# eddyxzc/lpopc

Measured on AMD Instinct MI355X. Metric: eval_g+eval_jac_g calls/sec, 4-phase 4096-LGR-pt problem, higher is better.
Workload: dtype f64

## Files before the change

lpopc_amd/csrc/rpm_abi.cpp:

```cpp
#include <cmath>
#include <cstdio>
#include <cstring>
#include <vector>
#include <new>
#include <string>

#include "rpm_engine.hpp"
#include "rpm_pin.h"

static thread_local std::string g_create_error;

using rpm::Engine;

#define RPM_GUARD_BEGIN try {
#define RPM_GUARD_END(eng)                                   \
  }                                                          \
  catch (const std::exception& ex) {                         \
    (eng).err = std::string("internal error: ") + ex.what(); \
    return RPM_E_INVALID;                                    \
  }                                                          \
  catch (...) {                                              \
    (eng).err = "internal error";                            \
    return RPM_E_INVALID;                                    \
  }

static int fail(Engine& e, int code, const char* msg) {
  e.err = msg;
  return code;
}

extern "C" {

int rpm_create(const rpm_problem_desc* desc, rpm_engine** out) {
  if (!out) {
    g_create_error = "rpm_create: out is NULL";
    return RPM_E_INVALID;
  }
  *out = nullptr;
  rpm_engine* h = new (std::nothrow) rpm_engine();
  if (!h) {
    g_create_error = "out of memory";
    return RPM_E_INVALID;
  }
  int rc;
  try {
    rc = rpm::setup_engine(h->e, desc);
  } catch (const std::exception& ex) {
    h->e.err = std::string("internal error: ") + ex.what();
    rc = RPM_E_INVALID;
  }
  if (rc != RPM_OK) {
    g_create_error = h->e.err;
    delete h;
    return rc;
  }
  *out = h;
  return RPM_OK;
}

void rpm_destroy(rpm_engine* h) {
  if (!h) return;
  rpm::device_destroy(h->e);
  delete h;
}

const char* rpm_last_error(const rpm_engine* h) {
  if (!h) return g_create_error.c_str();
  if (h->e.pin_note.empty()) return h->e.err.c_str();
  rpm_engine* w = const_cast<rpm_engine*>(h);
  w->e.err_report = h->e.err + (h->e.err.empty() ? "" : "; ") + "page-lock registry: " + h->e.pin_note;
  return w->e.err_report.c_str();
}

int rpm_device_init(rpm_engine* h, int device_id) {
  if (!h) return RPM_E_INVALID;
  RPM_GUARD_BEGIN
  return rpm::device_init(h->e, device_id);
  RPM_GUARD_END(h->e)
}

int rpm_get_nlp_info(rpm_engine* h, int* n, int* m, int* nnz_jac_g, int* nnz_h_lag, int* index_style) {
  if (!h) return RPM_E_INVALID;
  Engine& e = h->e;
  RPM_GUARD_BEGIN
  if (e.hessian_mode == RPM_HESSIAN_EXACT && nnz_h_lag) {
    int rc = rpm::ensure_hessian(e);
    if (rc) return rc;
  }
  if (n) *n = e.n;
  if (m) *m = e.m;
  if (nnz_jac_g) *nnz_jac_g = e.nnz_jac;
  if (nnz_h_lag) *nnz_h_lag = e.nnz_h;
  if (index_style) *index_style = 0;
  return RPM_OK;
  RPM_GUARD_END(e)
}

int rpm_get_bounds_info(rpm_engine* h, int n, double* x_l, double* x_u, int m, double* g_l, double* g_u) {
  if (!h) return RPM_E_INVALID;
  Engine& e = h->e;
  if (n != e.n || m != e.m || !x_l || !x_u || !g_l || !g_u) return fail(e, RPM_E_INVALID, "get_bounds_info: size mismatch");
  std::memcpy(x_l, e.xl.data(), sizeof(double) * e.n);
  std::memcpy(x_u, e.xu.data(), sizeof(double) * e.n);
  std::memcpy(g_l, e.gl.data(), sizeof(double) * e.m);
  std::memcpy(g_u, e.gu.data(), sizeof(double) * e.m);
  return RPM_OK;
}

int rpm_get_starting_point(rpm_engine* h, int n, int init_x, double* x, int init_z, double* z_L, double* z_U,
                           int m, int init_lambda, double* lambda) {
  (void)z_L; (void)z_U; (void)lambda;
  if (!h) return RPM_E_INVALID;
  Engine& e = h->e;
  if (!init_x || init_z || init_lambda) return fail(e, RPM_E_INVALID, "get_starting_point: only init_x is supported");
  if (n != e.n || m != e.m || !x) return fail(e, RPM_E_INVALID, "get_starting_point: size mismatch");
  std::memcpy(x, e.guess.data(), sizeof(double) * e.n);
  return RPM_OK;
}

static int stage_x(Engine& e, int n, const double* x) {
  if (n != e.n || !x) return fail(e, RPM_E_INVALID, "x size mismatch");
  if (!e.dev) {
    int rc = rpm::device_init(e, 0);
    if (rc) return rc;
  }
  return rpm::dev_upload_x(e, x);
}

int rpm_eval_f(rpm_engine* h, int n, const double* x, int new_x, double* obj_value) {
  if (!h) return RPM_E_INVALID;
  Engine& e = h->e;
  RPM_GUARD_BEGIN
  if (!obj_value) return fail(e, RPM_E_INVALID, "eval_f: obj_value is NULL");
  if (n != e.n || !x) return fail(e, RPM_E_INVALID, "x size mismatch");
  return rpm::host_eval_f(e, x, new_x, obj_value);
  RPM_GUARD_END(e)
}

int rpm_eval_grad_f(rpm_engine* h, int n, const double* x, int new_x, double* grad_f) {
  if (!h) return RPM_E_INVALID;
  Engine& e = h->e;
  RPM_GUARD_BEGIN
  if (!grad_f) return fail(e, RPM_E_INVALID, "eval_grad_f: grad_f is NULL");
  if (n != e.n || !x) return fail(e, RPM_E_INVALID, "x size mismatch");
  return rpm::host_eval_grad_f(e, x, new_x, grad_f);
  RPM_GUARD_END(e)
}

int rpm_eval_g(rpm_engine* h, int n, const double* x, int new_x, int m, double* g) {
  if (!h) return RPM_E_INVALID;
  Engine& e = h->e;
  RPM_GUARD_BEGIN
  if (n != e.n || !x) return fail(e, RPM_E_INVALID, "x size mismatch");
  if (m != e.m || !g) return fail(e, RPM_E_INVALID, "eval_g: size mismatch");
  return rpm::host_eval_g(e, x, new_x, g);
  RPM_GUARD_END(e)
}

int rpm_eval_jac_g(rpm_engine* h, int n, const double* x, int new_x, int m, int nele_jac, int* iRow, int* jCol,
                   double* values) {
  if (!h) return RPM_E_INVALID;
  Engine& e = h->e;
  RPM_GUARD_BEGIN
  if (n != e.n || m != e.m || nele_jac != e.nnz_jac) return fail(e, RPM_E_INVALID, "eval_jac_g: size mismatch");
  if (!values) {
    if (!iRow || !jCol) return fail(e, RPM_E_INVALID, "eval_jac_g: iRow/jCol are NULL in the structure pass");
    std::memcpy(iRow, e.jac_i.data(), sizeof(int) * e.nnz_jac);
    std::memcpy(jCol, e.jac_j.data(), sizeof(int) * e.nnz_jac);
    return RPM_OK;
  }
  if (!x) return fail(e, RPM_E_INVALID, "eval_jac_g: x is NULL");
  return rpm::host_eval_jac_values(e, x, new_x, values);
  RPM_GUARD_END(e)
}

int rpm_eval_pair(rpm_engine* h, int n, const double* x, int m, double* g, int nele_jac, double* values) {
  if (!h) return RPM_E_INVALID;
  Engine& e = h->e;
  RPM_GUARD_BEGIN
  if (n != e.n || m != e.m || nele_jac != e.nnz_jac || !x || !g || !values) return fail(e, RPM_E_INVALID, "eval_pair: size mismatch or NULL pointer");
  return rpm::host_eval_pair(e, x, g, values);
  RPM_GUARD_END(e)
}

int rpm_eval_h(rpm_engine* h, int n, const double* x, int new_x, double obj_factor, int m, const double* lambda,
               int new_lambda, int nele_hess, int* iRow, int* jCol, double* values) {
  (void)new_lambda;
  if (!h) return RPM_E_INVALID;
  Engine& e = h->e;
  RPM_GUARD_BEGIN
  if (e.hessian_mode != RPM_HESSIAN_EXACT) return fail(e, RPM_E_UNSUPPORTED, "eval_h: the engine was created with hessian-approximation=limited-memory");
  int rc = rpm::ensure_hessian(e);
  if (rc) return rc;
  if (n != e.n || m != e.m || nele_hess != e.nnz_h) return fail(e, RPM_E_INVALID, "eval_h: size mismatch");
  if (!values) {
    if (!iRow || !jCol) return fail(e, RPM_E_INVALID, "eval_h: iRow/jCol are NULL in the structure pass");
    std::memcpy(iRow, e.hes_i.data(), sizeof(int) * e.nnz_h);
    std::memcpy(jCol, e.hes_j.data(), sizeof(int) * e.nnz_h);
    return RPM_OK;
  }
  if (!x || !lambda) return fail(e, RPM_E_INVALID, "eval_h: x or lambda is NULL");
  if (new_x) rpm::host_new_x(e);
  rc = stage_x(e, n, x);
  if (rc) return rc;
  rc = rpm::dev_upload(e, rpm::dev_buf(e, 5), lambda, size_t(e.n_instances) * e.m, rpm::STAGE_LAMBDA);
  if (rc) return rc;
  rc = rpm::dev_eval_h(e, rpm::dev_buf(e, 0), obj_factor, rpm::dev_buf(e, 5), rpm::dev_buf(e, 6), rpm::dev_stream(e));
  if (rc) return rc;
  rc = rpm::dev_download(e, values, rpm::dev_buf(e, 6), size_t(e.n_instances) * e.nnz_h, rpm::STAGE_HESS);
  if (rc) return rc;
  if (e.opt_check_finite && rpm::dev_nonfinite(e, rpm::dev_buf(e, 6), size_t(e.n_instances) * e.nnz_h) != 0) return fail(e, RPM_E_NONFINITE, "eval_h: non-finite Hessian value");
  return RPM_OK;
  RPM_GUARD_END(e)
}

int rpm_finalize_solution(rpm_engine* h, int status, int n, const double* x, const double* z_L, const double* z_U,
                          int m, const double* g, const double* lambda, double obj_value) {
  (void)status; (void)z_L; (void)z_U; (void)g;
  if (!h) return RPM_E_INVALID;
  Engine& e = h->e;
  if (n != e.n || m != e.m || !x || !lambda) return fail(e, RPM_E_INVALID, "finalize_solution: size mismatch");
  e.sol_x.assign(x, x + n);
  e.sol_lambda.assign(lambda, lambda + m);
  e.sol_obj = obj_value;
  e.has_solution = true;
  return RPM_OK;
}

int rpm_get_solution(rpm_engine* h, int n, double* x, int m, double* lambda, double* obj_value) {
  if (!h) return RPM_E_INVALID;
  Engine& e = h->e;
  if (!e.has_solution) return fail(e, RPM_E_INVALID, "no solution stored");
  if (n != e.n || m != e.m) return fail(e, RPM_E_INVALID, "get_solution: size mismatch");
  if (x) std::memcpy(x, e.sol_x.data(), sizeof(double) * n);
  if (lambda) std::memcpy(lambda, e.sol_lambda.data(), sizeof(double) * m);
  if (obj_value) *obj_value = e.sol_obj;
  return RPM_OK;
}

int rpm_nlp2op_control(rpm_engine* h, int phase, const double* x, const double* lambda, double* time, double* state,
                       double* control, double* costate, double* pathmult, double* hamiltonian, double* mayer_cost,
                       double* lagrange_cost) {
  if (!h) return RPM_E_INVALID;
  Engine& e = h->e;
  RPM_GUARD_BEGIN
  if (phase < 0 || phase >= e.P) return fail(e, RPM_E_INVALID, "The phase index is out of rang");
  if (e.n_instances != 1) return fail(e, RPM_E_UNSUPPORTED, "nlp2op_control: one instance per engine");
  if (!x || !lambda) {
    if (!e.has_solution) return fail(e, RPM_E_INVALID, "nlp2op_control: no x/lambda given and no solution stored");
    x = e.sol_x.data();
    lambda = e.sol_lambda.data();
  }
  return rpm::dev_nlp2op(e, phase, x, lambda, time, state, control, costate, pathmult, hamiltonian, mayer_cost, lagrange_cost);
  RPM_GUARD_END(e)
}

int rpm_solution_error(rpm_engine* h, int phase, const double* x, double* rel_err, int* rows) {
  if (!h) return RPM_E_INVALID;
  Engine& e = h->e;
  RPM_GUARD_BEGIN
  if (phase < 0 || phase >= e.P) return fail(e, RPM_E_INVALID, "The phase index is out of rang");
  if (e.n_instances != 1) return fail(e, RPM_E_UNSUPPORTED, "solution_error: one instance per engine");
  if (!x) {
    if (!e.has_solution) return fail(e, RPM_E_INVALID, "solution_error: no x given and no solution stored");
    x = e.sol_x.data();
  }
  if (rows) *rows = e.ph[phase].N + e.ph[phase].K + 1;
  if (!rel_err) return RPM_OK;
  return rpm::dev_solution_error(e, phase, x, rel_err);
  RPM_GUARD_END(e)
}

static int refine_from(Engine& e, int phase, const double* rel, double tol, int nmin, int nmax, int capacity,
                       double* new_mesh_points, int* new_nodes_per_interval, int* new_n_intervals, double* interval_error,
                       int* no_more_refine) {
  std::vector<double> mesh, emax;
  std::vector<int> nodes;
  const bool done = rpm::ph_refine(e.ph[phase], rel, tol, nmin, nmax, mesh, nodes, emax);
  if (new_n_intervals) *new_n_intervals = int(nodes.size());
  if (no_more_refine) *no_more_refine = done ? 1 : 0;
  if (interval_error) std::memcpy(interval_error, emax.data(), sizeof(double) * emax.size());
  if (new_mesh_points || new_nodes_per_interval) {
    if (capacity < int(nodes.size())) return fail(e, RPM_E_INVALID, "ph_refine_mesh: capacity is smaller than the new interval count");
    if (new_mesh_points) std::memcpy(new_mesh_points, mesh.data(), sizeof(double) * mesh.size());
    if (new_nodes_per_interval) std::memcpy(new_nodes_per_interval, nodes.data(), sizeof(int) * nodes.size());
  }
  return RPM_OK;
}

int rpm_ph_refine_from_error(rpm_engine* h, int phase, const double* rel_err, double tol, int nmin, int nmax, int capacity,
                             double* new_mesh_points, int* new_nodes_per_interval, int* new_n_intervals,
                             double* interval_error, int* no_more_refine) {
  if (!h) return RPM_E_INVALID;
  Engine& e = h->e;
  RPM_GUARD_BEGIN
  if (phase < 0 || phase >= e.P) return fail(e, RPM_E_INVALID, "The phase index is out of rang");
  if (!rel_err) return fail(e, RPM_E_INVALID, "ph_refine_from_error: rel_err is NULL");
  if (!(tol > 0) || nmin < 2 || nmax < nmin) return fail(e, RPM_E_INVALID, "ph_refine_mesh: need tol > 0 and 2 <= Nmin <= Nmax");
  return refine_from(e, phase, rel_err, tol, nmin, nmax, capacity, new_mesh_points, new_nodes_per_interval, new_n_intervals,
                     interval_error, no_more_refine);
  RPM_GUARD_END(e)
}

int rpm_ph_refine_mesh(rpm_engine* h, int phase, const double* x, double tol, int nmin, int nmax, int capacity,
                       double* new_mesh_points, int* new_nodes_per_interval, int* new_n_intervals,
                       double* interval_error, int* no_more_refine) {
  if (!h) return RPM_E_INVALID;
  Engine& e = h->e;
  RPM_GUARD_BEGIN
  if (phase < 0 || phase >= e.P) return fail(e, RPM_E_INVALID, "The phase index is out of rang");
  if (e.n_instances != 1) return fail(e, RPM_E_UNSUPPORTED, "ph_refine_mesh: one instance per engine");
  if (!(tol > 0) || nmin < 2 || nmax < nmin) return fail(e, RPM_E_INVALID, "ph_refine_mesh: need tol > 0 and 2 <= Nmin <= Nmax");
  if (!x) {
    if (!e.has_solution) return fail(e, RPM_E_INVALID, "ph_refine_mesh: no x given and no solution stored");
    x = e.sol_x.data();
  }
  const rpm::PhaseHost& p = e.ph[phase];
  std::vector<double> rel(size_t(p.N + p.K + 1) * p.nx);
  int rc = rpm::dev_solution_error(e, phase, x, rel.data());
  if (rc) return rc;
  return refine_from(e, phase, rel.data(), tol, nmin, nmax, capacity, new_mesh_points, new_nodes_per_interval,
                     new_n_intervals, interval_error, no_more_refine);
  RPM_GUARD_END(e)
}

int rpm_solution_error_batch_sizes(rpm_engine* h, int* n_intervals_total, long long* rel_doubles_total) {
  if (!h) return RPM_E_INVALID;
  rpm::solution_error_batch_sizes(h->e, n_intervals_total, rel_doubles_total);
  return RPM_OK;
}

int rpm_solution_error_batch_dev(rpm_engine* h, const double* d_x, const int* d_instance_mask, double* d_interval_error,
                                 double* d_rel_err_max, double* d_rel_err, int* d_nonfinite, void* stream) {
  if (!h) return RPM_E_INVALID;
  Engine& e = h->e;
  RPM_GUARD_BEGIN
  if (!d_x) return fail(e, RPM_E_INVALID, "solution_error_batch_dev: d_x is NULL");
  if (e.shard_mode == RPM_SHARD_INTERVALS && e.shard_world > 1) return fail(e, RPM_E_UNSUPPORTED, "solution_error_batch: not with interval sharding");
  return rpm::dev_solution_error_batch(e, d_x, d_instance_mask, d_interval_error, d_rel_err_max, d_rel_err, d_nonfinite, stream);
  RPM_GUARD_END(e)
}

int rpm_solution_error_batch(rpm_engine* h, const double* x, const int* instance_mask, double* interval_error,
                             double* rel_err_max, double* rel_err, int* nonfinite) {
  if (!h) return RPM_E_INVALID;
  Engine& e = h->e;
  RPM_GUARD_BEGIN
  if (!x) return fail(e, RPM_E_INVALID, "solution_error_batch: x is NULL");
  if (e.shard_mode == RPM_SHARD_INTERVALS && e.shard_world > 1) return fail(e, RPM_E_UNSUPPORTED, "solution_error_batch: not with interval sharding");
  if (instance_mask && rel_err_max) {
    bool any = false;
    for (int b = 0; b < e.n_instances; ++b) any = any || instance_mask[b] != 0;
    if (!any) return fail(e, RPM_E_INVALID, "solution_error_batch: rel_err_max asked for, but instance_mask excludes every instance");
  }
  return rpm::host_solution_error_batch(e, x, instance_mask, interval_error, rel_err_max, rel_err, nonfinite);
  RPM_GUARD_END(e)
}

struct rpm_hpliu {
  rpm::HpLiu h;
  int n_phases = 0;
  std::string err;
};

int rpm_hpliu_create(int n_phases, double tol, int nmax, double ratio_r, rpm_hpliu** out) {
  if (!out || n_phases < 1 || !(tol > 0) || nmax < 2 || !(ratio_r > 0)) return RPM_E_INVALID;
  rpm_hpliu* p = new (std::nothrow) rpm_hpliu();
  if (!p) return RPM_E_INVALID;
  p->n_phases = n_phases;
  p->h.tol = tol;
  p->h.Nmax = nmax;
  p->h.R = ratio_r;
  *out = p;
  return RPM_OK;
}

void rpm_hpliu_destroy(rpm_hpliu* p) { delete p; }

const char* rpm_hpliu_last_error(const rpm_hpliu* p) { return p ? p->err.c_str() : "null hp-Liu object"; }

int rpm_hpliu_refine(rpm_hpliu* p, rpm_engine* h, const double* x, const double* rel_err, int capacity,
                     double* new_mesh_points, int* new_nodes_per_interval, int* mesh_off, int* nodes_off,
                     int* new_n_intervals, int* no_more_refine) {
  if (!p || !h) return RPM_E_INVALID;
  Engine& e = h->e;
  RPM_GUARD_BEGIN
  if (e.P != p->n_phases) return fail(e, RPM_E_INVALID, "hpliu_refine: phase count differs from rpm_hpliu_create");
  if (e.n_instances != 1) return fail(e, RPM_E_UNSUPPORTED, "hpliu_refine: one instance per engine");
  if (!x) {
    if (!e.has_solution) return fail(e, RPM_E_INVALID, "hpliu_refine: no x given and no solution stored");
    x = e.sol_x.data();
  }
  std::vector<std::vector<double>> rel(e.P);
  const double* src = rel_err;
  for (int ip = 0; ip < e.P; ++ip) {
    const rpm::PhaseHost& ph = e.ph[ip];
    const size_t cnt = size_t(ph.N + ph.K + 1) * ph.nx;
    rel[ip].resize(cnt);
    if (src) {
      std::memcpy(rel[ip].data(), src, cnt * sizeof(double));
      src += cnt;
    } else {
      int rc = rpm::dev_solution_error(e, ip, x, rel[ip].data());
      if (rc) return rc;
    }
  }
  std::vector<std::vector<double>> mesh;
  std::vector<std::vector<int>> nodes;
  bool done = false;
  int rc = p->h.refine(e, x, rel, mesh, nodes, &done, &p->err);
  if (rc) return fail(e, rc, p->err.c_str());
  int moff = 0, noff = 0;
  for (int ip = 0; ip < e.P; ++ip) {
    const int nk = int(nodes[ip].size());
    if (moff + nk + 1 > capacity || noff + nk > capacity) return fail(e, RPM_E_INVALID, "hpliu_refine: capacity too small for the new meshes (the refinement itself has been recorded)");
    std::memcpy(new_mesh_points + moff, mesh[ip].data(), sizeof(double) * (nk + 1));
    std::memcpy(new_nodes_per_interval + noff, nodes[ip].data(), sizeof(int) * nk);
    mesh_off[ip] = moff;
    nodes_off[ip] = noff;
    new_n_intervals[ip] = nk;
    moff += nk + 1;
    noff += nk;
  }
  if (no_more_refine) *no_more_refine = done ? 1 : 0;
  return RPM_OK;
  RPM_GUARD_END(e)
}

int rpm_final_result_save(rpm_engine* h, const char* dir) {
  if (!h) return RPM_E_INVALID;
  Engine& e = h->e;
  RPM_GUARD_BEGIN
  if (!e.has_solution) return fail(e, RPM_E_INVALID, "final_result_save: no solution stored (call rpm_finalize_solution first)");
  const std::string base = (dir && *dir) ? std::string(dir) + "/" : std::string();
  for (int ip = 0; ip < e.P; ++ip) {
    const rpm::PhaseHost& p = e.ph[ip];
    const int M = p.N + 1;
    std::vector<double> t(M), st(size_t(M) * p.nx), ct(size_t(M) * (p.nu ? p.nu : 1)), cs(size_t(M) * p.nx), ham(M);
    int rc = rpm::dev_nlp2op(e, ip, e.sol_x.data(), e.sol_lambda.data(), t.data(), st.data(), ct.data(), cs.data(), nullptr,
                             ham.data(), nullptr, nullptr);
    if (rc) return rc;
    auto save = [&](const char* stem, const double* a, int rows, int cols) -> bool {
      FILE* f = std::fopen((base + stem + std::to_string(ip + 1)).c_str(), "w");
      if (!f) return false;
      for (int r = 0; r < rows; ++r) {
        for (int c = 0; c < cols; ++c) std::fprintf(f, " %24.16e", a[r + size_t(c) * rows]);
        std::fputc('\n', f);
      }
      std::fclose(f);
      return true;
    };
    if (!save("time", t.data(), M, 1) || !save("state", st.data(), M, p.nx) || !save("control", ct.data(), M, p.nu) ||
        !save("parameter", e.sol_x.data() + p.var0 + p.nx * (p.N + 1) + p.nu * p.N + 2, p.nq, 1) ||
 !save("costate", cs.data(), M, p.nx) || !save("Hamiltonian", ham.data(), M, 1))
      return fail(e, RPM_E_INVALID, "final_result_save: cannot write the result files");
  }
  return RPM_OK;
  RPM_GUARD_END(e)
}

int rpm_eval_g_dev(rpm_engine* h, const double* d_x, double* d_g, void* stream) {
  if (!h) return RPM_E_INVALID;
  RPM_GUARD_BEGIN
  if (!d_x || !d_g) return fail(h->e, RPM_E_INVALID, "eval_g_dev: NULL pointer");
  return rpm::dev_eval_cons(h->e, d_x, d_g, nullptr, 1 | 4, stream);
  RPM_GUARD_END(h->e)
}
int rpm_eval_jac_g_dev(rpm_engine* h, const double* d_x, double* d_values, void* stream) {
  if (!h) return RPM_E_INVALID;
  RPM_GUARD_BEGIN
  if (!d_x || !d_values) return fail(h->e, RPM_E_INVALID, "eval_jac_g_dev: NULL pointer");
  return rpm::dev_eval_cons(h->e, d_x, nullptr, d_values, 2 | 4 | (h->e.opt_persistent_values ? 16 : 0), stream);
  RPM_GUARD_END(h->e)
}
int rpm_eval_pair_dev(rpm_engine* h, const double* d_x, double* d_g, double* d_values, void* stream) {
  if (!h) return RPM_E_INVALID;
  RPM_GUARD_BEGIN
  if (!d_x || !d_g || !d_values) return fail(h->e, RPM_E_INVALID, "eval_pair_dev: NULL pointer");
  return rpm::dev_eval_cons(h->e, d_x, d_g, d_values, 3 | 4 | (h->e.opt_persistent_values ? 16 : 0), stream);
  RPM_GUARD_END(h->e)
}
int rpm_eval_f_dev(rpm_engine* h, const double* d_x, double* d_obj, void* stream) {
  if (!h) return RPM_E_INVALID;
  RPM_GUARD_BEGIN
  if (!d_x || !d_obj) return fail(h->e, RPM_E_INVALID, "eval_f_dev: NULL pointer");
  return rpm::dev_eval_obj(h->e, d_x, d_obj, nullptr, stream);
  RPM_GUARD_END(h->e)
}
int rpm_eval_grad_f_dev(rpm_engine* h, const double* d_x, double* d_grad_f, void* stream) {
  if (!h) return RPM_E_INVALID;
  RPM_GUARD_BEGIN
  if (!d_x || !d_grad_f) return fail(h->e, RPM_E_INVALID, "eval_grad_f_dev: NULL pointer");
  return rpm::dev_eval_obj(h->e, d_x, nullptr, d_grad_f, stream);
  RPM_GUARD_END(h->e)
}
int rpm_eval_h_dev(rpm_engine* h, const double* d_x, double obj_factor, const double* d_lambda, double* d_values,
                   void* stream) {
  if (!h) return RPM_E_INVALID;
  RPM_GUARD_BEGIN
  if (h->e.hessian_mode != RPM_HESSIAN_EXACT) return fail(h->e, RPM_E_UNSUPPORTED, "eval_h_dev: the engine was created with hessian-approximation=limited-memory");
  if (!d_x || !d_lambda || !d_values) return fail(h->e, RPM_E_INVALID, "eval_h_dev: NULL pointer");
  return rpm::dev_eval_h(h->e, d_x, obj_factor, d_lambda, d_values, stream);
  RPM_GUARD_END(h->e)
}
int rpm_synchronize(rpm_engine* h) {
  if (!h) return RPM_E_INVALID;
  return rpm::dev_sync(h->e);
}

int rpm_set_instance_constants(rpm_engine* h, int instance, const double* consts, int n) {
  if (!h || !consts) return RPM_E_INVALID;
  RPM_GUARD_BEGIN
  Engine& e = h->e;
  if (instance < 0 || instance >= e.n_instances) return fail(e, RPM_E_INVALID, "rpm_set_instance_constants: instance out of range");
  if (n != int(e.consts.size())) return fail(e, RPM_E_INVALID, ("rpm_set_instance_constants: the problem functor takes " + std::to_string(e.consts.size()) + " constants").c_str());
  if (e.shard_world > 1) return fail(e, RPM_E_UNSUPPORTED, "rpm_set_instance_constants: not with interval sharding");
  if (n == 0) return RPM_OK;
  if (e.inst_consts.empty()) {
    e.inst_consts.resize(size_t(e.n_instances) * n);
    for (int b = 0; b < e.n_instances; ++b) std::copy(e.consts.begin(), e.consts.end(), e.inst_consts.begin() + size_t(b) * n);
  }
  std::copy(consts, consts + n, e.inst_consts.begin() + size_t(instance) * n);
  if (instance == 0) std::copy(consts, consts + n, e.consts.begin());
  return rpm::dev_update_instance_constants(e);
  RPM_GUARD_END(h->e)
}

int rpm_set_option(rpm_engine* h, const char* key, int value) {
  if (!h || !key) return RPM_E_INVALID;
  Engine& e = h->e;
  const std::string k(key);
  if (k == "fuse_pair") e.opt_fuse_pair = value ? 1 : 0;
  else if (k == "check_finite") e.opt_check_finite = value ? 1 : 0;
  else if (k == "pin_host") {
    e.opt_pin_host = value ? 1 : 0;
    e.pin_refused.clear();
    if (!value) {
      if (e.dev) { int rc = rpm::dev_sync(e); if (rc) return rc; }
      rpm::dev_pin_release_all(e);
    }
  }
  else if (k == "dx_mode") {
    if (value != 0 && value != 1) return fail(e, RPM_E_INVALID, "dx_mode must be 0 (scalar, reference order) or 1 (MFMA)");
    if (value == 1 && e.first_derive == RPM_DERIVE_ANALYTIC)
      return fail(e, RPM_E_UNSUPPORTED, "dx_mode=1 is only built for first-derive=finite-difference");
    e.opt_dx_mode = value;
  } else if (k == "tile_nodes") {
    if (value != 0 && value != 16 && value != 32 && value != 64) return fail(e, RPM_E_INVALID, "tile_nodes must be 0, 16, 32 or 64");
    if (e.dev) return fail(e, RPM_E_INVALID, "tile_nodes must be set before the device is initialised");
    e.opt_tile_nodes = value;
    if (value) {
      e.role_looped = false;
      rpm::build_tiles(e, value);
    }
  } else if (k == "instance_align") {
    if (value < 1 || value > 65536 || (value & (value - 1))) return fail(e, RPM_E_INVALID, "instance_align must be a power of two between 1 and 65536 doubles");
    if (e.ipm_attached > 0 && value != e.opt_instance_align)
      return fail(e, RPM_E_INVALID, "instance_align cannot change while an rpm_ipm solver is attached to the engine (its buffers are sized from the strides)");
    e.opt_instance_align = value;
  } else if (k == "const_once") {
    if (value != 0 && value != 1) return fail(e, RPM_E_INVALID, "const_once must be 0 or 1");
    e.opt_const_once = value;
    e.const_filled = nullptr;
  } else if (k == "ipm_local_border") {
    if (e.ipm_attached > 0) return fail(e, RPM_E_INVALID, "ipm_local_border must be set before rpm_ipm_create");
    e.opt_ipm_local_border = value != 0.0;
  } else if (k == "ipm_nested_group") {
    if (value < 0) return fail(e, RPM_E_INVALID, "ipm_nested_group must be >= 0 (0 = automatic)");
    if (e.ipm_attached > 0) return fail(e, RPM_E_INVALID, "ipm_nested_group must be set before rpm_ipm_create");
    e.opt_ipm_nested_group = value;
  } else if (k == "ipm_nested") {
    if (value < -1 || value > 1) return fail(e, RPM_E_INVALID, "ipm_nested must be -1 (automatic), 0 or 1");
    if (e.ipm_attached > 0) return fail(e, RPM_E_INVALID, "ipm_nested must be set before rpm_ipm_create");
    e.opt_ipm_nested = value;
  } else if (k == "persistent_values") {
    if (value != 0 && value != 1) return fail(e, RPM_E_INVALID, "persistent_values must be 0 or 1");
    e.opt_persistent_values = value;
  } else if (k == "delta_values") {
    if (value != 0 && value != 1) return fail(e, RPM_E_INVALID, "delta_values must be 0 or 1");
    e.opt_delta_values = value;
  } else if (k == "zero_copy") {
    if (value != 0 && value != 1) return fail(e, RPM_E_INVALID, "zero_copy must be 0 or 1");
    e.opt_zero_copy = value;
  } else if (k == "mesh_err_tile") {
    if (value != 0 && value != 1 && value != 2 && value != 4 && value != 8 && value != 16) return fail(e, RPM_E_INVALID, "mesh_err_tile must be 0 (auto), 1, 2, 4, 8 or 16");
    e.opt_mesh_err_tile = value;
  } else if (k == "pipeline") {
    if (value < -1 || value > 1) return fail(e, RPM_E_INVALID, "pipeline must be -1 (auto), 0 or 1");
    e.opt_pipeline = value;
  } else if (k == "stage_roles") {
    if (value < -1 || value > 1) return fail(e, RPM_E_INVALID, "stage_roles must be -1 (auto), 0 or 1");
    e.opt_stage_roles = value;
  } else if (k == "role_loop") {
    if (value < -1 || value > 1) return fail(e, RPM_E_INVALID, "role_loop must be -1 (auto), 0 or 1");
    if (e.dev) return fail(e, RPM_E_INVALID, "role_loop must be set before the device is initialised");
    e.opt_role_loop = value;
    if (e.opt_tile_nodes == 0) {
      long long total = 0;
      for (int i = 0; i < e.P; ++i) total += e.ph[i].N;
      total *= e.n_instances;
      e.role_looped = value == 1 || (value == -1 && total / 64 >= 512);
      rpm::build_tiles(e, e.role_looped ? 64 : 16);
    }
  } else
    return fail(e, RPM_E_INVALID, "unknown option");
  rpm::host_new_x(e);
  rpm::dev_forget_persistent(e);
  return RPM_OK;
}
int rpm_get_option(rpm_engine* h, const char* key, int* value) {
  if (!h || !key || !value) return RPM_E_INVALID;
  Engine& e = h->e;
  const std::string k(key);
  if (k == "fuse_pair") *value = e.opt_fuse_pair;
  else if (k == "check_finite") *value = e.opt_check_finite;
  else if (k == "dx_mode") *value = e.opt_dx_mode;
  else if (k == "tile_nodes") *value = e.tile_nodes;
  else if (k == "n_tiles") *value = int(e.tiles.size());
  else if (k == "role_loop") *value = e.role_looped ? 1 : 0;
  else if (k == "pipeline") *value = e.opt_pipeline;
  else if (k == "mesh_err_tile") *value = e.opt_mesh_err_tile;
  else if (k == "stage_roles") *value = e.opt_stage_roles;
  else if (k == "const_once") *value = e.opt_const_once;
  else if (k == "instance_align") *value = e.opt_instance_align;
  else if (k == "delta_values") *value = e.opt_delta_values;
  else if (k == "ipm_nested") *value = e.opt_ipm_nested;
  else if (k == "ipm_nested_group") *value = e.opt_ipm_nested_group;
  else if (k == "ipm_local_border") *value = e.opt_ipm_local_border;
  else if (k == "zero_copy") *value = e.opt_zero_copy;
  else if (k == "persistent_values") *value = e.opt_persistent_values;
  else if (k == "pin_host") *value = e.opt_pin_host;
  else if (k == "pin_registered") *value = int(rpm::dev_pin_counter(RPM_PIN_REGISTERED));
  else if (k == "pin_register_failures") *value = int(rpm::dev_pin_counter(RPM_PIN_REGISTER_FAILURES));
  else if (k == "pin_unregistered") *value = int(rpm::dev_pin_counter(RPM_PIN_UNREGISTERED));
  else if (k == "pin_unregister_failures") *value = int(rpm::dev_pin_counter(RPM_PIN_UNREGISTER_FAILURES));
  else if (k == "pin_overlap_refused") *value = int(rpm::dev_pin_counter(RPM_PIN_OVERLAP_REFUSED));
  else if (k == "pin_shared") *value = int(rpm::dev_pin_counter(RPM_PIN_SHARED));
  else if (k == "pin_merged") *value = int(rpm::dev_pin_counter(RPM_PIN_MERGED));
  else if (k == "pin_evicted") *value = int(rpm::dev_pin_counter(RPM_PIN_EVICTED));
  else if (k == "pin_live") *value = int(rpm::dev_pin_counter(RPM_PIN_LIVE));
  else if (k == "pin_live_kb") *value = int(rpm::dev_pin_counter(RPM_PIN_LIVE_BYTES) / 1024);
  else if (k == "pin_held") *value = rpm::dev_pin_held(e);
  else if (k == "delta_sent_runs") return rpm::host_delta_sent_runs(e, value);
  else if (k == "delta_total_runs") *value = e.last_delta_total;
  else if (k == "stride_g") *value = int(e.stride_g());
  else if (k == "stride_values") *value = int(e.stride_values());
  else if (k == "pipeline_active") *value = rpm::dev_pipeline_active(e);
  else return fail(e, RPM_E_INVALID, "unknown option");
  return RPM_OK;
}

int rpm_get_phase_sizes(rpm_engine* h, int phase, int* n_nodes, int* d_nnz, int* doff_nnz) {
  if (!h) return RPM_E_INVALID;
  Engine& e = h->e;
  if (phase < 0 || phase >= e.P) return fail(e, RPM_E_INVALID, "The phase index is out of rang");
  if (n_nodes) *n_nodes = e.ph[phase].N;
  if (d_nnz) *d_nnz = int(e.ph[phase].d_v.size());
  if (doff_nnz) *doff_nnz = int(e.ph[phase].off_v.size());
  return RPM_OK;
}
int rpm_get_phase_tables(rpm_engine* h, int phase, double* points, double* weights, int* d_rows, int* d_cols,
                         double* d_vals, double* diag_vals, int* doff_rows, int* doff_cols, double* doff_vals) {
  if (!h) return RPM_E_INVALID;
  Engine& e = h->e;
  if (phase < 0 || phase >= e.P) return fail(e, RPM_E_INVALID, "The phase index is out of rang");
  const rpm::PhaseHost& p = e.ph[phase];
  auto cp = [](auto* dst, const auto& v) {
    if (dst && !v.empty()) std::memcpy(dst, v.data(), v.size() * sizeof(v[0]));
  };
  cp(points, p.points);
  cp(weights, p.weights);
  cp(d_rows, p.d_i);
  cp(d_cols, p.d_j);
  cp(d_vals, p.d_v);
  cp(diag_vals, p.diag_v);
  cp(doff_rows, p.off_i);
  cp(doff_cols, p.off_j);
  cp(doff_vals, p.off_v);
  return RPM_OK;
}

int rpm_shard_segments(rpm_engine* h, int which, int rank, rpm_segment* seg, int* n_seg, int* packed_len) {
  if (!h) return RPM_E_INVALID;
  Engine& e = h->e;
  RPM_GUARD_BEGIN
  if (which < 0 || which > 1 || rank < 0 || rank >= e.shard_world) return fail(e, RPM_E_INVALID, "shard_segments: bad argument");
  int plen = 0;
  std::vector<rpm_segment> s = rpm::shard_segments(e, which, rank, &plen);
  if (seg) {
    if (!n_seg || *n_seg < int(s.size())) return fail(e, RPM_E_INVALID, "shard_segments: segment buffer too small");
    std::memcpy(seg, s.data(), s.size() * sizeof(rpm_segment));
  }
  if (n_seg) *n_seg = int(s.size());
  if (packed_len) *packed_len = plen;
  return RPM_OK;
  RPM_GUARD_END(e)
}
int rpm_shard_pack_dev(rpm_engine* h, int which, const double* d_full, double* d_packed, void* stream) {
  if (!h) return RPM_E_INVALID;
  RPM_GUARD_BEGIN
  if (!d_full || !d_packed || which < 0 || which > 1) return fail(h->e, RPM_E_INVALID, "shard_pack_dev: bad argument");
  return rpm::dev_shard_copy(h->e, which, true, d_full, 0, d_packed, stream);
  RPM_GUARD_END(h->e)
}
int rpm_shard_unpack_dev(rpm_engine* h, int which, const double* d_gathered, int stride, double* d_full, void* stream) {
  if (!h) return RPM_E_INVALID;
  RPM_GUARD_BEGIN
  if (!d_gathered || !d_full || which < 0 || which > 1) return fail(h->e, RPM_E_INVALID, "shard_unpack_dev: bad argument");
  return rpm::dev_shard_copy(h->e, which, false, d_gathered, stride, d_full, stream);
  RPM_GUARD_END(h->e)
}
int rpm_shard_slot_len(rpm_engine* h, long long* slot_doubles) {
  if (!h || !slot_doubles) return RPM_E_INVALID;
  RPM_GUARD_BEGIN
  *slot_doubles = rpm::shard_slot_len(h->e);
  return RPM_OK;
  RPM_GUARD_END(h->e)
}
int rpm_shard_pack_all_dev(rpm_engine* h, const double* d_g, const double* d_values, double* d_slot, void* stream) {
  if (!h) return RPM_E_INVALID;
  RPM_GUARD_BEGIN
  if (!d_g || !d_values || !d_slot) return fail(h->e, RPM_E_INVALID, "shard_pack_all_dev: NULL pointer");
  return rpm::dev_shard_pack_all(h->e, d_g, d_values, d_slot, stream);
  RPM_GUARD_END(h->e)
}
int rpm_shard_unpack_all_dev(rpm_engine* h, const double* d_gathered, double* d_g, double* d_values, int skip_own, void* stream) {
  if (!h) return RPM_E_INVALID;
  RPM_GUARD_BEGIN
  if (!d_g || !d_values || !d_gathered) return fail(h->e, RPM_E_INVALID, "shard_unpack_all_dev: NULL pointer");
  return rpm::dev_shard_unpack_all(h->e, d_gathered, d_g, d_values, skip_own, stream);
  RPM_GUARD_END(h->e)
}
}
```

lpopc_amd/csrc/rpm_device.hip:

```cpp
#include "rpm_device_internal.hpp"
#include "rpm_pin.h"

namespace rpm {

template <class Prob, bool GRAD, bool AN>
__global__ void rpm_obj_kernel(const KParams K, const double* __restrict__ xall, double* __restrict__ objall,
                               double* __restrict__ gradall, double* __restrict__ partial) {
  constexpr int NX = Prob::NX, NU = Prob::NU, NQ = prob_nq<Prob>::value;
  constexpr int NXs = NX > 0 ? NX : 1, NUs = NU > 0 ? NU : 1, NQs = NQ > 0 ? NQ : 1;
  __shared__ double red[2 + NQs][256];
  const int tid = threadIdx.x;
  const int p = blockIdx.x;
  const int inst = blockIdx.y;
  const double* __restrict__ x = xall + size_t(inst) * K.n;
  double* grad = GRAD ? gradall + size_t(inst) * K.n : nullptr;
  const PhaseDev ph = K.phases[p];
  const double* c = K.consts + size_t(inst) * K.consts_stride;
  const int N = ph.N;
  bool bad = false;
  const double t0 = x[ph.x_t0], tf = x[ph.x_t0 + 1];
  const double tspan = tf - t0;
  double s_wl = 0.0, s_t0 = 0.0;
  double s_p[NQs];
  double pq[NQs];
#pragma unroll
  for (int j = 0; j < NQs; ++j) { s_p[j] = 0.0; pq[j] = j < NQ ? x[ph.x_t0 + 2 + j] : 0.0; }
  for (int k = tid; k < N; k += blockDim.x) {
    const double tau = K.points[ph.node0 + k], w = K.weights[ph.node0 + k];
    const double tk = (tau + 1) * (tspan / 2.0) + t0;
    double xs[NXs], us[NUs];
#pragma unroll
    for (int i = 0; i < NX; ++i) xs[i] = x[ph.x_state0 + i * (N + 1) + k];
#pragma unroll
    for (int j = 0; j < NU; ++j) us[j] = x[ph.x_control0 + j * N + k];
    const double L0 = pf_lagrange<Prob>(ph.phase_num, tk, xs, us, pq, c);
    s_wl += w * L0;
    if (GRAD) {
      const double wk = w * tspan / 2.0;
      double dLt;
      if constexpr (AN) {
#pragma unroll
        for (int i = 0; i < NX; ++i)
          { const double gv_ = wk * pf_lagrange_grad_col<Prob>(ph.phase_num, i, tk, xs, us, pq, c); grad[ph.x_state0 + i * (N + 1) + k] = gv_; chk_note(bad, gv_); }
#pragma unroll
        for (int j = 0; j < NU; ++j)
          { const double gv_ = wk * pf_lagrange_grad_col<Prob>(ph.phase_num, NX + j, tk, xs, us, pq, c); grad[ph.x_control0 + j * N + k] = gv_; chk_note(bad, gv_); }
        dLt = pf_lagrange_grad_col<Prob>(ph.phase_num, NX + NU, tk, xs, us, pq, c);
#pragma unroll
        for (int j = 0; j < NQ; ++j) s_p[j] += wk * pf_lagrange_grad_col<Prob>(ph.phase_num, NX + NU + 1 + j, tk, xs, us, pq, c);
      } else {
#pragma unroll
        for (int i = 0; i < NX; ++i) {
          const double b = xs[i], hh = K.tol * (1 + fabs(b));
          xs[i] = b + hh;
          const double Lp = pf_lagrange<Prob>(ph.phase_num, tk, xs, us, pq, c);
          xs[i] = b;
          { const double gv_ = wk * ((Lp - L0) / hh); grad[ph.x_state0 + i * (N + 1) + k] = gv_; chk_note(bad, gv_); }
        }
#pragma unroll
        for (int j = 0; j < NU; ++j) {
          const double b = us[j], hh = K.tol * (1 + fabs(b));
          us[j] = b + hh;
          const double Lp = pf_lagrange<Prob>(ph.phase_num, tk, xs, us, pq, c);
          us[j] = b;
          { const double gv_ = wk * ((Lp - L0) / hh); grad[ph.x_control0 + j * N + k] = gv_; chk_note(bad, gv_); }
        }
        const double ht = K.tol * (1 + fabs(tk));
        dLt = (pf_lagrange<Prob>(ph.phase_num, tk + ht, xs, us, pq, c) - L0) / ht;
#pragma unroll
        for (int j = 0; j < NQ; ++j) {
          const double b = pq[j], hh = K.tol * (1 + fabs(b));
          pq[j] = b + hh;
          const double Lp = pf_lagrange<Prob>(ph.phase_num, tk, xs, us, pq, c);
          pq[j] = b;
          s_p[j] += wk * ((Lp - L0) / hh);
        }
      }
      s_t0 += ((w * (tspan / 2.0)) * dLt) * (tau * (-0.5) + 0.5);
    }
  }
  red[0][tid] = s_wl;
  red[1][tid] = s_t0;
#pragma unroll
  for (int j = 0; j < NQ; ++j) red[2 + j][tid] = s_p[j];
  __syncthreads();
  for (int s = blockDim.x / 2; s > 0; s >>= 1) {
    if (tid < s) {
      red[0][tid] += red[0][tid + s];
      red[1][tid] += red[1][tid + s];
#pragma unroll
      for (int j = 0; j < NQ; ++j) red[2 + j][tid] += red[2 + j][tid + s];
    }
    __syncthreads();
  }
  if (tid == 0) {
    double x0[NXs], xf[NXs];
#pragma unroll
    for (int i = 0; i < NX; ++i) {
      x0[i] = x[ph.x_state0 + i * (N + 1)];
      xf[i] = x[ph.x_state0 + i * (N + 1) + N];
    }
    const double wl = red[0][0];
    const double mayer = pf_mayer<Prob>(ph.phase_num, t0, x0, tf, xf, pq, c);
    partial[size_t(inst) * K.P + p] = mayer + wl * (tspan / 2.0);
    if (GRAD) {
      double dM[2 * NXs + 2 + NQs];
      if constexpr (AN) {
        for (int q = 0; q < 2 * NX + 2 + NQ; ++q) dM[q] = pf_mayer_grad_col<Prob>(ph.phase_num, q, t0, x0, tf, xf, pq, c);
      } else {
        const double m0 = mayer;
        const double h0 = K.tol * (1 + fabs(t0)), hf = K.tol * (1 + fabs(tf));
        dM[NX] = (pf_mayer<Prob>(ph.phase_num, t0 + h0, x0, tf, xf, pq, c) - m0) / h0;
        dM[2 * NX + 1] = (pf_mayer<Prob>(ph.phase_num, t0, x0, tf + hf, xf, pq, c) - m0) / hf;
        for (int j = 0; j < NQ; ++j) {
          const double b = pq[j], hb = K.tol * (1 + fabs(b));
          pq[j] = b + hb;
          dM[2 * NX + 2 + j] = (pf_mayer<Prob>(ph.phase_num, t0, x0, tf, xf, pq, c) - m0) / hb;
          pq[j] = b;
        }
        for (int i = 0; i < NX; ++i) {
          const double b0 = x0[i], hb0 = K.tol * (1 + fabs(b0));
          x0[i] = b0 + hb0;
          dM[i] = (pf_mayer<Prob>(ph.phase_num, t0, x0, tf, xf, pq, c) - m0) / hb0;
          x0[i] = b0;
          const double bf = xf[i], hbf = K.tol * (1 + fabs(bf));
          xf[i] = bf + hbf;
          dM[NX + 1 + i] = (pf_mayer<Prob>(ph.phase_num, t0, x0, tf, xf, pq, c) - m0) / hbf;
          xf[i] = bf;
        }
      }
      for (int i = 0; i < NX; ++i) { const double gv_ = dM[NX + 1 + i]; grad[ph.x_state0 + i * (N + 1) + N] = gv_; chk_note(bad, gv_); }
      { const double gv_ = (red[1][0] + dM[NX]) + (-0.5) * wl; grad[ph.x_t0] = gv_; chk_note(bad, gv_); }
      double dLt0;
      {
        double xs[NXs], us[NUs];
        for (int i = 0; i < NX; ++i) xs[i] = x0[i];
        for (int j = 0; j < NU; ++j) us[j] = x[ph.x_control0 + j * N];
        const double tau = K.points[ph.node0];
        const double tk = (tau + 1) * (tspan / 2.0) + t0;
        if constexpr (AN) {
          dLt0 = pf_lagrange_grad_col<Prob>(ph.phase_num, NX + NU, tk, xs, us, pq, c);
        } else {
          const double ht = K.tol * (1 + fabs(tk));
          dLt0 = (pf_lagrange<Prob>(ph.phase_num, tk + ht, xs, us, pq, c) - pf_lagrange<Prob>(ph.phase_num, tk, xs, us, pq, c)) / ht;
        }
        const double r2 = (K.weights[ph.node0] * (tspan / 2.0)) * dLt0;
        { const double gv_ = (dM[2 * NX + 1] + 0.5 * wl) + (tau * 0.5 + 0.5) * r2; grad[ph.x_t0 + 1] = gv_; chk_note(bad, gv_); }
      }
      for (int j = 0; j < NQ; ++j) { const double gv_ = dM[2 * NX + 2 + j] + red[2 + j][0]; grad[ph.x_t0 + 2 + j] = gv_; chk_note(bad, gv_); }
    }
  }
  (void)objall;
  if (GRAD && K.chk != nullptr && bad) atomicOr_system(K.chk + 3, 1);
}

__global__ void rpm_obj_sum_kernel(int P, int B, const double* __restrict__ partial, double* __restrict__ obj) {
  const int inst = blockIdx.x * blockDim.x + threadIdx.x;
  if (inst >= B) return;
  double cost = 0.0;
  for (int p = 0; p < P; ++p) cost += partial[size_t(inst) * P + p];
  obj[inst] = cost;
}

bool problem_dims(int id, ProblemDims* out) {
  return with_problem(id, [&](auto prob) {
    using P = decltype(prob);
    *out = ProblemDims{P::NX, P::NU, P::NC, P::NE_MAX, P::NLINK_MAX, P::NCONST, P::HAS_ANALYTIC, prob_nq<P>::value};
  });
}

void device_destroy(Engine& e) {
  Device* d = e.dev;
  if (!d) return;
  (void)hipSetDevice(d->device_id);
#ifdef RPM_DIAG
  if (d->kp.trace) {
    (void)hipDeviceSynchronize();
    std::vector<unsigned long long> h(d->trace_words);
    (void)hipMemcpy(h.data(), d->kp.trace, d->trace_words * 8, hipMemcpyDeviceToHost);
    if (FILE* f = std::fopen(getenv("RPM_DIAG_TRACE"), "wb")) {
      std::fwrite(h.data(), 8, h.size(), f);
      std::fclose(f);
    }
    (void)hipFree(d->kp.trace);
  }
#endif
  void* ptrs[] = {d->d_phases, d->d_tiles, d->d_tasks, d->d_nodes, d->d_points, d->d_weights, d->d_diag,
                  d->d_dvals, d->d_doff, d->d_consts, d->d_inst_consts, d->d_alin_v, d->d_links, d->d_alin_j, d->d_x, d->d_g,
                  d->d_values, d->d_grad, d->d_obj, d->d_lambda, d->d_hess, d->d_partial, d->d_hpairs, d->d_hphases,
                  d->d_hends, d->d_hlinks, d->d_htiles, d->d_htmp};
  for (void* p : ptrs)
    if (p) (void)hipFree(p);
  if (d->d_flag) (void)hipFree(d->d_flag);
  if (d->h_flags2) (void)hipHostFree(d->h_flags2);
  host_path_destroy(d);
  exchange_destroy(d);
  mesh_batch_destroy(d);
  rpm_pin_release_owner(&e);
  dev_stage_destroy(d);
  for (auto& row : d->segtab)
    for (auto& t : row)
      if (t.ptr) (void)hipFree(t.ptr);
  if (d->stream) (void)hipStreamDestroy(d->stream);
  delete d;
  e.dev = nullptr;
}

int device_init(Engine& e, int device_id) {
  if (e.dev) {
    if (e.dev->device_id == device_id) return RPM_OK;
    device_destroy(e);
  }
  int count = 0;
  hipError_t s = hipGetDeviceCount(&count);
  if (s != hipSuccess || count <= 0) {
    e.err = "no HIP device available (this engine has no CPU fallback)";
    return RPM_E_DEVICE;
  }
  if (device_id < 0 || device_id >= count) {
    e.err = "device id out of range";
    return RPM_E_DEVICE;
  }
  HIP_TRY(e, hipSetDevice(device_id));
  Device* d = new Device();
  e.dev = d;
  d->device_id = device_id;
  HIP_TRY(e, hipStreamCreateWithFlags(&d->stream, hipStreamNonBlocking));
  HIP_TRY(e, upload(&d->d_phases, e.phd));
  {
    std::vector<TileDev> mine;
    for (int id : e.my_tiles) mine.push_back(e.tiles[id]);
    HIP_TRY(e, upload(&d->d_tiles, mine));
  }
  HIP_TRY(e, upload(&d->d_tasks, e.tasks));
  HIP_TRY(e, upload(&d->d_nodes, e.nodes));
  HIP_TRY(e, upload(&d->d_points, e.points));
  HIP_TRY(e, upload(&d->d_weights, e.weights));
  HIP_TRY(e, upload(&d->d_diag, e.diag));
  HIP_TRY(e, upload(&d->d_dvals, e.dvals));
  HIP_TRY(e, upload(&d->d_doff, e.doff_vals));
  HIP_TRY(e, upload(&d->d_consts, e.consts));
  HIP_TRY(e, upload(&d->d_links, e.links));
  HIP_TRY(e, upload(&d->d_alin_j, e.alin_j));
  HIP_TRY(e, upload(&d->d_alin_v, e.alin_v));
  const size_t B = size_t(e.n_instances);
  HIP_TRY(e, hipMalloc(reinterpret_cast<void**>(&d->d_x), B * e.n * sizeof(double)));
  HIP_TRY(e, hipMalloc(reinterpret_cast<void**>(&d->d_g), B * e.m * sizeof(double)));
  HIP_TRY(e, hipMalloc(reinterpret_cast<void**>(&d->d_values), B * size_t(e.nnz_jac) * sizeof(double)));
  HIP_TRY(e, hipMalloc(reinterpret_cast<void**>(&d->d_grad), B * e.n * sizeof(double)));
  HIP_TRY(e, hipMalloc(reinterpret_cast<void**>(&d->d_obj), B * sizeof(double)));
  HIP_TRY(e, hipMalloc(reinterpret_cast<void**>(&d->d_partial), B * e.P * sizeof(double)));
  HIP_TRY(e, hipMalloc(reinterpret_cast<void**>(&d->d_lambda), B * e.m * sizeof(double)));
  HIP_TRY(e, hipMemsetAsync(d->d_grad, 0, B * e.n * sizeof(double), d->stream));
  KParams& k = d->kp;
  k.phases = d->d_phases;
  k.tiles = d->d_tiles;
  k.n_my_tiles = int(e.my_tiles.size());
  k.nodes = d->d_nodes;
  k.points = d->d_points;
  k.weights = d->d_weights;
  k.diag = d->d_diag;
  k.dvals = d->d_dvals;
  k.doff_vals = d->d_doff;
  k.consts = d->d_consts;
  k.consts_stride = 0;
  k.links = d->d_links;
  k.alin_j = d->d_alin_j;
  k.alin_v = d->d_alin_v;
  k.tol = e.fd_tol;
  k.P = e.P;
  k.L = e.L;
  k.n = e.n;
  k.m = e.m;
  k.m_nl = e.m_nl;
  k.nnz = e.nnz_jac;
  k.nnz_nl = e.nnz_nl;
  k.nnz_lin = e.nnz_lin;
  k.nnz_const = e.nnz_const;
  k.max_span = e.max_span;
  k.max_drow = e.max_drow;
  k.sg = e.m;
  k.sv = e.nnz_jac;
  k.max_cshare = 0;
  for (const TileDev& t : e.tiles) k.max_cshare = t.c_cnt > k.max_cshare ? t.c_cnt : k.max_cshare;
  const bool sharded = e.shard_mode == RPM_SHARD_INTERVALS && e.shard_world > 1;
  k.tasks = d->d_tasks;
  k.n_tasks = (!sharded || e.shard_rank == 0) ? int(e.tasks.size()) : 0;
  k.skip_const = 0;
  k.trace = nullptr;
  k.chk = nullptr;
#ifdef RPM_DIAG
  if (getenv("RPM_DIAG_TRACE")) {
    size_t words = size_t(e.tiles.size() * 2 + e.tasks.size() + 64) * size_t(e.n_instances) * 8;
    if (words < size_t(4096) * 64) words = size_t(4096) * 64;
    if (hipMalloc(reinterpret_cast<void**>(&k.trace), words * 8) == hipSuccess) (void)hipMemset(k.trace, 0, words * 8);
    d->trace_words = words;
  }
#endif
  ProblemDims pd;
  problem_dims(e.problem_id, &pd);
  d->lds_bytes = size_t(std::max(TileLds(pd.nx, pd.nu, pd.nc, e.tile_nodes, e.max_span, e.max_drow).total, 64)) * sizeof(double);
  if (d->lds_bytes > 160 * 1024) {
    e.err = "mesh interval too large for the LDS-staged D tile (reduce nodes per interval)";
    return RPM_E_UNSUPPORTED;
  }
  tile_pipeline_setup(e, d, pd, device_id);
  return dev_update_instance_constants(e);
}

int dev_eval_obj(Engine& e, const double* d_x, double* d_obj, double* d_grad, void* stream, bool host_chk) {
  if (!e.dev) {
    int rc = device_init(e, 0);
    if (rc) return rc;
  }
  Device& dd = *e.dev;
  struct { KParams kp; double* d_partial; } d{dd.kp, dd.d_partial};
  d.kp.chk = host_chk ? dd.d_flags2 : nullptr;
  hipStream_t st = static_cast<hipStream_t>(stream);
  const bool an = e.first_derive == RPM_DERIVE_ANALYTIC;
  hipError_t s = hipSuccess;
  with_problem(e.problem_id, [&](auto prob) {
    using P = decltype(prob);
    dim3 grid(unsigned(e.P), unsigned(e.n_instances));
    if (d_grad) {
      bool done = false;
      if constexpr (P::HAS_ANALYTIC) {
        if (an) {
          hipLaunchKernelGGL((rpm_obj_kernel<P, true, true>), grid, dim3(256), 0, st, d.kp, d_x, d_obj, d_grad, d.d_partial);
          done = true;
        }
      }
      if (!done)
        hipLaunchKernelGGL((rpm_obj_kernel<P, true, false>), grid, dim3(256), 0, st, d.kp, d_x, d_obj, d_grad, d.d_partial);
    } else {
      hipLaunchKernelGGL((rpm_obj_kernel<P, false, false>), grid, dim3(256), 0, st, d.kp, d_x, d_obj, d_grad, d.d_partial);
    }
    s = hipGetLastError();
  });
  if (s == hipSuccess && d_obj) {
    const int B = e.n_instances;
    const int thr = B < 256 ? B : 256;
    hipLaunchKernelGGL(rpm_obj_sum_kernel, dim3(unsigned((B + thr - 1) / thr)), dim3(unsigned(thr)), 0, st, e.P, B,
                       d.d_partial, d_obj);
    s = hipGetLastError();
  }
  if (s != hipSuccess) {
    e.err = std::string("rpm_obj_kernel launch: ") + hipGetErrorString(s);
    return RPM_E_DEVICE;
  }
  return RPM_OK;
}

__global__ void rpm_finite_kernel(const double* __restrict__ v, size_t n, int* __restrict__ flag) {
  bool bad = false;
  for (size_t i = size_t(blockIdx.x) * blockDim.x + threadIdx.x; i < n; i += size_t(gridDim.x) * blockDim.x)
    bad |= !isfinite(v[i]);
  if (__any(bad) && (threadIdx.x & 63) == 0) atomicOr(flag, 1);
}

int dev_nonfinite(Engine& e, const double* dev, size_t count) {
  Device& d = *e.dev;
  if (!d.d_flag) {
    if (hipMalloc(reinterpret_cast<void**>(&d.d_flag), sizeof(int)) != hipSuccess) return -1;
  }
  if (hipMemsetAsync(d.d_flag, 0, sizeof(int), d.stream) != hipSuccess) return -1;
  unsigned blocks = unsigned((count + 255) / 256);
  if (blocks > 2048) blocks = 2048;
  if (blocks == 0) blocks = 1;
  hipLaunchKernelGGL(rpm_finite_kernel, dim3(blocks), dim3(256), 0, d.stream, dev, count, d.d_flag);
  int h = 0;
  if (hipMemcpyAsync(&h, d.d_flag, sizeof(int), hipMemcpyDeviceToHost, d.stream) != hipSuccess) return -1;
  if (hipStreamSynchronize(d.stream) != hipSuccess) return -1;
  return h;
}

__global__ void rpm_finite2_kernel(const double* __restrict__ a, size_t na, const double* __restrict__ b, size_t nb,
                                   int* __restrict__ flags) {
  bool bad_a = false, bad_b = false;
  const size_t stride = size_t(gridDim.x) * blockDim.x, first = size_t(blockIdx.x) * blockDim.x + threadIdx.x;
  for (size_t i = first; i < na; i += stride) bad_a |= !isfinite(a[i]);
  for (size_t i = first; i < nb; i += stride) bad_b |= !isfinite(b[i]);
  if (__any(bad_a) && (threadIdx.x & 63) == 0) atomicOr_system(flags, 1);
  if (__any(bad_b) && (threadIdx.x & 63) == 0) atomicOr_system(flags + 1, 1);
}

int dev_nonfinite_enqueue(Engine& e, const double* a, size_t na, const double* b, size_t nb) {
  Device& d = *e.dev;
  if (!d.h_flags2) {
    if (hipHostMalloc(reinterpret_cast<void**>(&d.h_flags2), 4 * sizeof(int), hipHostMallocMapped) != hipSuccess) return RPM_E_DEVICE;
    d.h_flags2[2] = d.h_flags2[3] = 0;
    if (hipHostGetDevicePointer(reinterpret_cast<void**>(&d.d_flags2), d.h_flags2, 0) != hipSuccess) return RPM_E_DEVICE;
  }
  d.h_flags2[0] = d.h_flags2[1] = 0;
  const size_t most = na > nb ? na : nb;
  unsigned blocks = unsigned((most + 255) / 256);
  if (blocks > 8192) blocks = 8192;
  if (blocks == 0) blocks = 1;
  hipLaunchKernelGGL(rpm_finite2_kernel, dim3(blocks), dim3(256), 0, d.stream, a, na, b, nb, d.d_flags2);
  return RPM_OK;
}
int dev_flag_value(Engine& e, int slot) { return e.dev->h_flags2 ? e.dev->h_flags2[slot] : 0; }

constexpr int PIN_MAX = 8;
long dev_pin_counter(int which) { return rpm_pin_counter(which); }
int dev_pin_held(const Engine& e) { return rpm_pin_held(&e); }
void dev_pin_release_all(Engine& e) {
  rpm_pin_release_owner(&e);
  e.pin_refused.clear();
}
std::string dev_pin_last_error() {
  char buf[320];
  buf[0] = 0;
  rpm_pin_last_error(buf, sizeof buf);
  return buf;
}
void* dev_pin_host(Engine& e, const void* ptr, size_t bytes) {
  const bool sharded = e.shard_mode == RPM_SHARD_INTERVALS && e.shard_world > 1;
  if (!e.opt_pin_host || !ptr || bytes == 0 || (bytes < RPM_PIN_MIN_BYTES && !sharded)) return nullptr;
  for (const auto& r : e.pin_refused)
    if (r.first == ptr && r.second == bytes) return nullptr;
  const long refused = rpm_pin_counter(RPM_PIN_REGISTER_FAILURES) + rpm_pin_counter(RPM_PIN_OVERLAP_REFUSED);
  void* alias = rpm_pin_acquire(&e, ptr, bytes, PIN_MAX, sharded ? 1 : 0);
  if (!alias && rpm_pin_counter(RPM_PIN_REGISTER_FAILURES) + rpm_pin_counter(RPM_PIN_OVERLAP_REFUSED) != refused)
    e.pin_note = dev_pin_last_error();
  if (!alias) {
    if (e.pin_refused.size() >= 16) e.pin_refused.erase(e.pin_refused.begin());
    e.pin_refused.emplace_back(ptr, bytes);
  }
  return alias;
}

int dev_stage_reserve(Engine& e, int slot, size_t count, double** host, double** alias) {
  Device& d = *e.dev;
  Device::Stage& s = d.stage[slot];
  if (s.busy || s.cap < count) {
    HIP_TRY(e, hipStreamSynchronize(d.stream));
    dev_stage_synced(e);
  }
  if (s.cap < count) {
    if (s.h) HIP_TRY(e, hipHostFree(s.h));
    s.h = s.d = nullptr;
    s.cap = 0;
    const size_t cap = count + count / 4 + 64;
    HIP_TRY(e, hipHostMalloc(reinterpret_cast<void**>(&s.h), cap * sizeof(double), hipHostMallocMapped));
    HIP_TRY(e, hipHostGetDevicePointer(reinterpret_cast<void**>(&s.d), s.h, 0));
    s.cap = cap;
  }
  *host = s.h;
  if (alias) *alias = s.d;
  return RPM_OK;
}
void dev_stage_synced(Engine& e) {
  if (!e.dev) return;
  for (Device::Stage& s : e.dev->stage) s.busy = false;
}
void dev_stage_destroy(Device* d) {
  for (Device::Stage& s : d->stage) {
    if (s.h) (void)hipHostFree(s.h);
    s = Device::Stage{};
  }
}
int dev_stage_upload(Engine& e, int slot, double* dev, const double* host, size_t count) {
  if (count == 0) return RPM_OK;
  if (dev_pin_host(e, host, count * sizeof(double))) {
    HIP_TRY(e, hipMemcpyAsync(dev, host, count * sizeof(double), hipMemcpyHostToDevice, e.dev->stream));
    HIP_TRY(e, hipStreamSynchronize(e.dev->stream));
    dev_stage_synced(e);
    return RPM_OK;
  }
  double* h = nullptr;
  int rc = dev_stage_reserve(e, slot, count, &h, nullptr);
  if (rc) return rc;
  std::memcpy(h, host, count * sizeof(double));
  HIP_TRY(e, hipMemcpyAsync(dev, h, count * sizeof(double), hipMemcpyHostToDevice, e.dev->stream));
  e.dev->stage[slot].busy = true;
  return RPM_OK;
}
int dev_stage_download(Engine& e, int slot, double* host, const double* dev, size_t count) {
  if (count == 0) return RPM_OK;
  if (dev_pin_host(e, host, count * sizeof(double))) {
    HIP_TRY(e, hipMemcpyAsync(host, dev, count * sizeof(double), hipMemcpyDeviceToHost, e.dev->stream));
    HIP_TRY(e, hipStreamSynchronize(e.dev->stream));
    dev_stage_synced(e);
    return RPM_OK;
  }
  double* h = nullptr;
  int rc = dev_stage_reserve(e, slot, count, &h, nullptr);
  if (rc) return rc;
  HIP_TRY(e, hipMemcpyAsync(h, dev, count * sizeof(double), hipMemcpyDeviceToHost, e.dev->stream));
  HIP_TRY(e, hipStreamSynchronize(e.dev->stream));
  dev_stage_synced(e);
  std::memcpy(host, h, count * sizeof(double));
  return RPM_OK;
}

int dev_upload_x(Engine& e, const double* x) {
  if (!e.dev) {
    int rc = device_init(e, 0);
    if (rc) return rc;
  }
  HIP_TRY(e, hipSetDevice(e.dev->device_id));
  return dev_stage_upload(e, STAGE_X, e.dev->d_x, x, size_t(e.n_instances) * e.n);
}
int dev_download(Engine& e, double* host, const double* dev, size_t count, int slot) {
  return dev_stage_download(e, slot, host, dev, count);
}
int dev_upload(Engine& e, double* dev, const double* host, size_t count, int slot) {
  return dev_stage_upload(e, slot, dev, host, count);
}
int dev_update_instance_constants(Engine& e) {
  if (!e.dev || e.inst_consts.empty()) return RPM_OK;
  Device& d = *e.dev;
  const size_t count = e.inst_consts.size();
  if (!d.d_inst_consts) HIP_TRY(e, hipMalloc(reinterpret_cast<void**>(&d.d_inst_consts), count * sizeof(double)));
  HIP_TRY(e, hipStreamSynchronize(d.stream));
  HIP_TRY(e, hipMemcpy(d.d_inst_consts, e.inst_consts.data(), count * sizeof(double), hipMemcpyHostToDevice));
  d.kp.consts = d.d_inst_consts;
  d.kp.consts_stride = int(e.consts.size());
  host_new_x(e);
  return RPM_OK;
}

int dev_sync(Engine& e) {
  if (!e.dev) return RPM_OK;
  HIP_TRY(e, hipStreamSynchronize(e.dev->stream));
  dev_stage_synced(e);
  return RPM_OK;
}
double* dev_buf(Engine& e, int which) {
  Device& d = *e.dev;
  switch (which) {
    case 0: return d.d_x;
    case 1: return d.d_g;
    case 2: return d.d_values;
    case 3: return d.d_grad;
    case 4: return d.d_obj;
    case 5: return d.d_lambda;
    case 6: return d.d_hess;
  }
  return nullptr;
}
bool& dev_cache_valid(Engine& e) { return e.dev->cache_valid; }
void dev_forget_persistent(Engine& e) {
  if (e.dev) e.dev->const_filled.clear();
}
void* dev_stream(Engine& e) { return e.dev->stream; }

struct SegCopy { int src, dst, len, pad; };
__global__ void rpm_seg_copy_kernel(const SegCopy* __restrict__ segs, const double* __restrict__ src,
                                    double* __restrict__ dst) {
  const SegCopy s = segs[blockIdx.x];
  for (int i = blockIdx.y * blockDim.x + threadIdx.x; i < s.len; i += gridDim.y * blockDim.x)
    dst[s.dst + i] = src[s.src + i];
}

int dev_shard_copy(Engine& e, int which, bool pack, const double* src, int stride, double* dst, void* stream) {
  if (!e.dev) {
    int rc = device_init(e, 0);
    if (rc) return rc;
  }
  Device& d = *e.dev;
  hipStream_t st = static_cast<hipStream_t>(stream);
  Device::SegTable& tab = d.segtab[which][pack ? 0 : 1];
  if (!tab.ptr || tab.stride != stride) {
    std::vector<SegCopy> segs;
    if (pack) {
      for (const rpm_segment& s : shard_segments(e, which, e.shard_rank, nullptr)) segs.push_back(SegCopy{s.off, s.pos, s.len, 0});
    } else {
      for (int r = 0; r < e.shard_world; ++r)
        for (const rpm_segment& s : shard_segments(e, which, r, nullptr)) segs.push_back(SegCopy{r * stride + s.pos, s.off, s.len, 0});
    }
    if (tab.ptr) HIP_TRY(e, hipFree(tab.ptr));
    tab.ptr = nullptr;
    tab.count = int(segs.size());
    tab.stride = stride;
    if (tab.count) {
      HIP_TRY(e, hipMalloc(&tab.ptr, segs.size() * sizeof(SegCopy)));
      HIP_TRY(e, hipMemcpy(tab.ptr, segs.data(), segs.size() * sizeof(SegCopy), hipMemcpyHostToDevice));
    }
  }
  if (!tab.count) return RPM_OK;
  hipLaunchKernelGGL(rpm_seg_copy_kernel, dim3(unsigned(tab.count), 4), dim3(256), 0, st,
                     static_cast<const SegCopy*>(tab.ptr), src, dst);
  HIP_TRY(e, hipGetLastError());
  return RPM_OK;
}

}
```

lpopc_amd/csrc/rpm_device_internal.hpp:

```cpp
#pragma once
#include <hip/hip_runtime.h>

#include <algorithm>
#include <cmath>
#include <cstdio>
#include <cstdlib>
#include <cstring>
#include <string>
#include <utility>
#include <vector>

#include "problems/problems.hpp"
#ifdef RPM_USER_PROBLEM_HEADER
#include RPM_USER_PROBLEM_HEADER
#endif
#include "rpm_engine.hpp"

namespace rpm {

struct KParams {
  const PhaseDev* phases;
  const TileDev* tiles;
  int n_my_tiles;
  const TaskDev* tasks;
  int n_tasks;
  const NodeDev* nodes;
  const double* points;
  const double* weights;
  const double* diag;
  const double* dvals;
  const double* doff_vals;
  const double* consts;
  int consts_stride;
  const LinkDev* links;
  const int* alin_j;
  const double* alin_v;
  double tol;
  int P, L, n, m, m_nl, nnz, nnz_nl, nnz_lin, nnz_const;
  long long sg, sv;
  int max_span, max_drow;
  int max_cshare;
  int skip_const;
  unsigned long long* trace;
  int* chk;
};

struct TileLds {
  int Xs;
  int Us;
  int Ds;
  int Fb;
  int DXs;
  int total;
  __host__ __device__ constexpr TileLds(int nx, int nu, int nc, int T, int max_span, int max_drow)
      : Xs(0), Us(Xs + nx * max_span), Ds(Us + nu * T), Fb(Ds + max_drow), DXs(Fb + (nx + nc) * T), total(DXs + nx * T) {}
};
constexpr bool tile_lds_pinned(int nx, int nu, int nc, int T, int span, int drow) {
  const TileLds L(nx, nu, nc, T, span, drow);
  return L.Xs == 0 && L.Us == L.Xs + nx * span && L.Ds == L.Us + nu * T && L.Fb == L.Ds + drow && L.DXs == L.Fb + (nx + nc) * T &&
         L.total == L.DXs + nx * T && L.total == nx * span + nu * T + drow + (nx + nc) * T + nx * T;
}
static_assert(tile_lds_pinned(LaunchProblem::NX, LaunchProblem::NU, LaunchProblem::NC, 64, 73, 64 * 9) &&
                  tile_lds_pinned(QuadrotorProblem::NX, QuadrotorProblem::NU, QuadrotorProblem::NC, 16, 40, 16 * 41),
              "TileLds: an array overlaps its neighbour or the total changed");

struct HParams {
  const HessPairDev* pairs;
  const HessPhaseDev* phases;
  const HessEndDev* ends;
  const HessLinkDev* links;
  const int* tiles;
  int n_tiles, th, n_ends, n_links, nnz_h, tmp_len;
};

struct Device {
  int device_id = -1;
  int* d_flags2 = nullptr;
  int* h_flags2 = nullptr;
  size_t trace_words = 0;
  hipStream_t stream = nullptr;
  KParams kp{};
  PhaseDev* d_phases = nullptr;
  TileDev* d_tiles = nullptr;
  TaskDev* d_tasks = nullptr;
  NodeDev* d_nodes = nullptr;
  double* d_inst_consts = nullptr;
  double *d_points = nullptr, *d_weights = nullptr, *d_diag = nullptr, *d_dvals = nullptr,
         *d_doff = nullptr, *d_consts = nullptr, *d_alin_v = nullptr;
  LinkDev* d_links = nullptr;
  int* d_alin_j = nullptr;
  double *d_x = nullptr, *d_g = nullptr, *d_values = nullptr, *d_grad = nullptr, *d_obj = nullptr,
         *d_lambda = nullptr, *d_hess = nullptr;
  double* d_partial = nullptr;
  int* d_flag = nullptr;
  struct Stage { double* h = nullptr; double* d = nullptr; size_t cap = 0; bool busy = false; };
  Stage stage[STAGE_SLOTS];
  bool cache_valid = false;
  std::vector<const double*> const_filled;
  size_t lds_bytes = 0;
  int pl_slots = 0;
  size_t pl_lds = 0;
  bool pl_ok = false;
  HessPairDev* d_hpairs = nullptr;
  HessPhaseDev* d_hphases = nullptr;
  HessEndDev* d_hends = nullptr;
  HessLinkDev* d_hlinks = nullptr;
  int* d_htiles = nullptr;
  double* d_htmp = nullptr;
  HParams hp{};
  size_t hess_lds = 0;
  int hess_threads = 0;
  void* host_path = nullptr;
  void* exchange = nullptr;
  void* mesh_batch = nullptr;
  struct SegTable { void* ptr = nullptr; int count = 0; int stride = -1; };
  SegTable segtab[2][2];
};

#define HIP_TRY(e, call)                                                                   \
  do {                                                                                     \
    hipError_t _s = (call);                                                                \
    if (_s != hipSuccess) {                                                                \
      (e).err = std::string(#call) + ": " + hipGetErrorString(_s);                         \
      return RPM_E_DEVICE;                                                                 \
    }                                                                                      \
  } while (0)

__device__ __forceinline__ void chk_note(bool& bad, double v) { bad |= !(fabs(v) <= 1.7976931348623157e308); }
__device__ __forceinline__ void chk_report(int* chk, bool bad_g, bool bad_j) {
  if (chk == nullptr) return;
  if (bad_g) atomicOr_system(chk, 1);
  if (bad_j) atomicOr_system(chk + 1, 1);
}

template <class F>
inline bool with_problem(int id, F&& fn) {
  switch (id) {
#ifndef RPM_ONLY_USER_PROBLEM
    case RPM_PROBLEM_LAUNCH: fn(LaunchProblem{}); return true;
    case RPM_PROBLEM_HYPERSENSITIVE: fn(HypersensitiveProblem{}); return true;
    case RPM_PROBLEM_BRYSON_DENHAM: fn(BrysonDenhamProblem{}); return true;
    case RPM_PROBLEM_BRACHISTOCHRONE: fn(BrachistochroneProblem{}); return true;
    case RPM_PROBLEM_MIN_TIME_CLIMB: fn(MinTimeClimbProblem{}); return true;
    case RPM_PROBLEM_QUADROTOR: fn(QuadrotorProblem{}); return true;
    case RPM_PROBLEM_PARAM_SLED: fn(ParamSledProblem{}); return true;
    case RPM_PROBLEM_PARAM_OSC: fn(ParamOscProblem{}); return true;
#endif
#ifdef RPM_USER_PROBLEM_HEADER
    case RPM_PROBLEM_USER: fn(UserProblem{}); return true;
#endif
  }
  return false;
}


template <class T>
inline hipError_t upload(T** dst, const std::vector<T>& src) {
  const size_t bytes = (src.size() ? src.size() : 1) * sizeof(T);
  hipError_t s = hipMalloc(reinterpret_cast<void**>(dst), bytes);
  if (s != hipSuccess) return s;
  if (!src.empty()) s = hipMemcpy(*dst, src.data(), src.size() * sizeof(T), hipMemcpyHostToDevice);
  return s;
}


void host_path_destroy(Device* d);
int dev_stage_reserve(Engine& e, int slot, size_t count, double** host, double** alias);
int dev_stage_upload(Engine& e, int slot, double* dev, const double* host, size_t count);
int dev_stage_download(Engine& e, int slot, double* host, const double* dev, size_t count);
void dev_stage_destroy(Device* d);
void host_new_x(Engine& e);
void dev_stage_synced(Engine& e);
std::string dev_pin_last_error();
void exchange_destroy(Device* d);
void mesh_batch_destroy(Device* d);

void tile_pipeline_setup(Engine& e, Device* d, const ProblemDims& pd, int device_id);

}
```

lpopc_amd/csrc/rpm_engine.hpp:

```cpp
#pragma once
#include <cstddef>
#include <string>
#include <utility>
#include <vector>

#include "../../include/rpm_hip.h"

namespace rpm {

struct PhaseDev {
  int N, nx, nu, nc, ne;
  int nq;
  int phase_num;
  int x_state0;
  int x_control0;
  int x_t0;
  int g0;
  int v_nl0;
  int v_evt0;
  int node0;
  int doff_base;
  int off_nnz;
  int const_cum;
  int tile0, ntiles;
};

struct TileDev {
  int phase;
  int k0, cnt;
  int span0, span_len;
  int drow0, drow_len;
  int N, phase_num, x_state0, x_control0, x_t0, g0, v_nl0, node0;
  int c_src0, c_cnt, c_dst0, c_stride, c_copies;
};

struct HessPairDev {
  int a, b;
  int kind;
  int dst0, dst1;
};
struct HessPhaseDev {
  int pair0;
  int v0;
  int nI, nE;
  int tt_dst[3];
  int end0, n_end;
  int tt_tmp;
};
struct HessEndDev { int phase, a, b, da, db, dst; };
struct HessLinkDev { int pair, a, b, dst; };

struct TaskDev { int type, idx; };

struct NodeDev {
  int drow_off;
  int dcol0;
  int dlen;
  int interval;
};

struct LinkDev {
  int left, right;
  int nlink;
  int g0;
  int v0;
};

struct MeshIvDev {
  int n;
  int istart;
  int r0;
  int q0;
  int hs, hc;
  int a;
};
struct MeshErrTables {
  std::vector<MeshIvDev> iv;
  std::vector<double> ttem, Hs, Ss, Hc, Sc, A;
  std::vector<int> hit_s, hit_c;
  int fine_nodes = 0, rows = 0;
};

struct PhaseHost {
  int nx = 0, nu = 0, nq = 0, nc = 0, ne = 0, K = 0, N = 0;
  std::vector<double> mesh;
  std::vector<int> nk;
  std::vector<double> points, weights;
  std::vector<int> d_i, d_j;
  std::vector<double> d_v;
  std::vector<double> diag_v;
  std::vector<int> off_i, off_j;
  std::vector<double> off_v;
  std::vector<double> drows;
  std::vector<NodeDev> nodes;
  int var0 = 0, con0 = 0, nvar = 0, ncon = 0;
};

enum { STAGE_X = 0, STAGE_G, STAGE_V, STAGE_GRAD, STAGE_LAMBDA, STAGE_HESS, STAGE_SLOTS };

struct Device;

struct Engine {
  int problem_id = 0, P = 0, L = 0;
  std::vector<double> consts;
  std::vector<double> inst_consts;
  double fd_tol = 1e-6;
  int first_derive = 0, hessian_mode = 0;
  int n_instances = 1;
  int shard_mode = 0, shard_rank = 0, shard_world = 1;
  std::vector<PhaseHost> ph;
  std::vector<LinkDev> links;
  std::vector<std::vector<double>> link_min, link_max;
  int n = 0, m_nl = 0, m = 0;
  int nnz_nl = 0, nnz_lin = 0, nnz_const = 0, nnz_jac = 0, nnz_h = 0;
  std::vector<double> xl, xu, gl, gu, guess;
  std::vector<int> alin_i, alin_j;
  std::vector<double> alin_v;
  std::vector<int> jac_i, jac_j;
  std::vector<int> hes_i, hes_j;
  bool hess_ready = false;
  std::vector<std::vector<int>> hess_dep;
  std::vector<HessPairDev> hess_pairs;
  std::vector<HessPhaseDev> hess_phases;
  std::vector<HessEndDev> hess_ends;
  std::vector<HessLinkDev> hess_links;
  int hess_tmp_len = 0;
  std::vector<PhaseDev> phd;
  std::vector<TileDev> tiles;
  std::vector<int> my_tiles;
  std::vector<TaskDev> tasks;
  std::vector<NodeDev> nodes;
  std::vector<double> points, weights, diag, dvals, doff_vals;
  int tile_nodes = 16;
  bool role_looped = false;
  int max_span = 0, max_drow = 0;
  int opt_fuse_pair = 1, opt_dx_mode = 0, opt_tile_nodes = 0, opt_check_finite = 1, opt_const_once = 0;
  int opt_role_loop = -1;
  int opt_instance_align = 1;
  long long stride_g() const { return (long long)(m + opt_instance_align - 1) / opt_instance_align * opt_instance_align; }
  long long stride_values() const { return (long long)(nnz_jac + opt_instance_align - 1) / opt_instance_align * opt_instance_align; }
  int opt_stage_roles = -1;
  int opt_pipeline = -1;
  int jac_nonfinite = -1;
  const double* const_filled = nullptr;
  int opt_persistent_values = 0;
  int opt_pin_host = 0;
  std::vector<std::pair<const void*, size_t>> pin_refused;
  std::string pin_note;
  int opt_zero_copy = 1;
  int opt_delta_values = 0;
  int last_delta_total = 0;
  int opt_ipm_nested_group = 0;
  int opt_ipm_local_border = 1;
  int opt_ipm_nested = -1;
  int opt_mesh_err_tile = 0;
  int ipm_attached = 0;
  std::vector<double> sol_x, sol_lambda;
  double sol_obj = 0.0;
  bool has_solution = false;
  std::vector<MeshErrTables> mesh_err;
  std::string err;
  std::string err_report;
  Device* dev = nullptr;
};

int setup_engine(Engine& e, const rpm_problem_desc* d);
void build_tiles(Engine& e, int tile_nodes);
void lgr_points(int n, std::vector<double>& x, std::vector<double>& w);
void colloc_d(const std::vector<double>& pts, std::vector<double>& D);

void build_hessian_tables(Engine& e);
int ensure_hessian(Engine& e);
int dev_eval_h(Engine& e, const double* d_x, double obj_factor, const double* d_lambda, double* d_values, void* stream);

int dev_nlp2op(Engine& e, int phase, const double* x, const double* lambda, double* time, double* state, double* control,
               double* costate, double* pathmult, double* hamiltonian, double* mayer_cost, double* lagrange_cost);

struct HpLiu {
  struct Mesh { std::vector<double> mesh; std::vector<int> nodes; std::vector<double> e_k; };
  struct Solution { int rows = 0; std::vector<double> v; };
  double tol = 1e-6, R = 1.2;
  int Nmax = 16, mesh_index = 0;
  std::vector<std::vector<Mesh>> meshes;
  std::vector<std::vector<Solution>> states;
  std::vector<std::vector<std::vector<double>>> points_hist;
  int refine(const Engine& e, const double* x, const std::vector<std::vector<double>>& rel,
             std::vector<std::vector<double>>& new_mesh, std::vector<std::vector<int>>& new_nodes, bool* no_more,
             std::string* why);
  int smooth_enough(int ip, int first_row, int n, const std::vector<double>& tau, const double* state, int ld, int nx) const;
  bool exponent(int ip, double m0, double mf, int N, double e_k, double* q) const;
};
void lagrange_rows(const double* src, int m, const double* dst, int nq, double* H, double* S, int* hit);

void build_mesh_err_tables(const PhaseHost& p, MeshErrTables& t);
bool ph_refine(const PhaseHost& p, const double* rel, double tol, int nmin, int nmax, std::vector<double>& mesh,
               std::vector<int>& nodes, std::vector<double>& interval_error);
int dev_solution_error(Engine& e, int phase, const double* x, double* rel_err);
void solution_error_batch_sizes(const Engine& e, int* n_intervals_total, long long* rel_doubles_total);
constexpr double mesh_err_max(double a, double v) { return (v > a || v != v) ? v : a; }
int dev_solution_error_batch(Engine& e, const double* d_x, const int* d_mask, double* d_interval_error, double* d_rel_err_max,
                             double* d_rel_err, int* d_nonfinite, void* stream);
int host_solution_error_batch(Engine& e, const double* x, const int* mask, double* interval_error, double* rel_err_max,
                              double* rel_err, int* nonfinite);

std::vector<rpm_segment> shard_segments(const Engine& e, int which, int rank, int* packed_len);
int dev_shard_copy(Engine& e, int which, bool pack, const double* src, int stride, double* dst, void* stream);
long long shard_slot_len(const Engine& e);
int dev_shard_pack_all(Engine& e, const double* d_g, const double* d_values, double* d_slot, void* stream);
int dev_shard_unpack_all(Engine& e, const double* d_gathered, double* d_g, double* d_values, int skip_own, void* stream);

struct ProblemDims { int nx, nu, nc, ne_max, nlink_max, nconst; bool has_analytic; int nq; };
bool problem_dims(int problem_id, ProblemDims* out);

int device_init(Engine& e, int device_id);
void device_destroy(Engine& e);
int dev_eval_cons(Engine& e, const double* d_x, double* d_g, double* d_values, int flags, void* stream);
int dev_eval_obj(Engine& e, const double* d_x, double* d_obj, double* d_grad, void* stream, bool host_chk = false);
bool dev_cons_is_one_role(const Engine& e);
int host_eval_f(Engine& e, const double* x, int new_x, double* obj);
int host_eval_grad_f(Engine& e, const double* x, int new_x, double* grad);
int host_eval_g(Engine& e, const double* x, int new_x, double* g);
void host_new_x(Engine& e);
int host_eval_jac_values(Engine& e, const double* x, int new_x, double* values);
int host_eval_pair(Engine& e, const double* x, double* g, double* values);
struct ConsCall { bool want_g, want_v, cached, delta, launched_jac; };
int host_cons_begin(Engine& e, const double* x, int new_x, double* g, double* values, ConsCall* c);
int host_cons_end(Engine& e, double* g, double* values, const ConsCall& c, const char* who);
int host_delta_sent_runs(Engine& e, int* sent);
int dev_pipeline_active(const Engine& e);
int dev_upload_x(Engine& e, const double* x);
int dev_upload(Engine& e, double* dev, const double* host, size_t count, int slot);
int dev_download(Engine& e, double* host, const double* dev, size_t count, int slot);
int dev_sync(Engine& e);
int dev_update_instance_constants(Engine& e);
double* dev_buf(Engine& e, int which);
bool& dev_cache_valid(Engine& e);
void dev_forget_persistent(Engine& e);
void* dev_stream(Engine& e);
int dev_nonfinite(Engine& e, const double* dev, size_t count);
int dev_nonfinite_enqueue(Engine& e, const double* a, size_t na, const double* b, size_t nb);
int dev_flag_value(Engine& e, int slot);
long dev_pin_counter(int which);
int dev_pin_held(const Engine& e);
void* dev_pin_host(Engine& e, const void* ptr, size_t bytes);
void dev_pin_release_all(Engine& e);

}

struct rpm_engine {
  rpm::Engine e;
};
```

lpopc_amd/csrc/rpm_tile_kernels.hip:

```cpp
#include "rpm_device_internal.hpp"

namespace rpm {


template <class Prob, bool WG, bool WJ, bool AN, bool WAVE = false>
__device__ void endpoint_block(const KParams& K, const TaskDev task, const double* __restrict__ x,
                               double* __restrict__ g, double* __restrict__ vals, double* lds, int inst) {
  constexpr int NX = Prob::NX, NQ = prob_nq<Prob>::value, NQs = NQ > 0 ? NQ : 1;
  bool bad_g = false, bad_j = false;
  constexpr int NE = Prob::NE_MAX > 0 ? Prob::NE_MAX : 1;
  constexpr int NL = Prob::NLINK_MAX > 0 ? Prob::NLINK_MAX : 1;
  static_assert(!WAVE || 2 * NX + 3 + 2 * NQ <= 64, "endpoint perturbations must fit one wave");
  const int tid = WAVE ? int(threadIdx.x & 63) : int(threadIdx.x);
  const int nthr = WAVE ? 64 : int(blockDim.x);
  const double* c = K.consts + size_t(inst) * K.consts_stride;
  if (task.type == 0) {
    for (int r = tid; r < K.P + K.L; r += nthr) {
      if (WG) {
        double acc = 0.0;
        acc += K.alin_v[2 * r] * x[K.alin_j[2 * r]];
        acc += K.alin_v[2 * r + 1] * x[K.alin_j[2 * r + 1]];
        g[K.m_nl + r] = acc;
        chk_note(bad_g, acc);
      }
      if (WJ) {
        vals[K.nnz_nl + 2 * r] = K.alin_v[2 * r];
        vals[K.nnz_nl + 2 * r + 1] = K.alin_v[2 * r + 1];
      }
    }
  } else if (task.type == 1) {
    const PhaseDev ph = K.phases[task.idx];
    const int pi = tid;
    const bool act = pi <= 2 * NX + 2 + NQ;
    double x0[NX], xf[NX], ev[NE], pp[NQs];
#pragma unroll
    for (int j = 0; j < NQ; ++j) pp[j] = x[ph.x_t0 + 2 + j];
    double t0 = x[ph.x_t0], tf = x[ph.x_t0 + 1];
#pragma unroll
    for (int j = 0; j < NX; ++j) {
      x0[j] = x[ph.x_state0 + j * (ph.N + 1)];
      xf[j] = x[ph.x_state0 + j * (ph.N + 1) + ph.N];
    }
    double h = 1.0;
    if (WJ && !AN && pi >= 1) {
      const int v = pi - 1;
#pragma unroll
      for (int j = 0; j < NX; ++j) {
        if (v == j) { h = K.tol * (fabs(x0[j]) + 1); x0[j] += h; }
        if (v == NX + 1 + j) { h = K.tol * (fabs(xf[j]) + 1); xf[j] += h; }
      }
      if (v == NX) { h = K.tol * (1 + fabs(t0)); t0 += h; }
      if (v == 2 * NX + 1) { h = K.tol * (1 + fabs(tf)); tf += h; }
#pragma unroll
      for (int j = 0; j < NQ; ++j)
        if (v == 2 * NX + 2 + j) { h = K.tol * (1 + fabs(pp[j])); pp[j] += h; }
    }
#pragma unroll
    for (int i = 0; i < NE; ++i) ev[i] = 0.0;
    if (act && (pi == 0 || !AN)) pf_event<Prob>(ph.phase_num, t0, x0, tf, xf, pp, c, ev);
    double base[NE];
    if constexpr (WAVE) {
#pragma unroll
      for (int i = 0; i < NE; ++i) base[i] = __shfl(ev[i], 0, 64);
    }
    if (pi == 0) {
#pragma unroll
      for (int i = 0; i < NE; ++i)
        if (i < ph.ne) {
          if (!WAVE) lds[i] = ev[i];
          if (WG) { g[ph.g0 + (NX + Prob::NC) * ph.N + i] = ev[i]; chk_note(bad_g, ev[i]); }
        }
    }
    if constexpr (!WAVE) {
      __syncthreads();
#pragma unroll
      for (int i = 0; i < NE; ++i) base[i] = lds[i];
    }
    if (WJ && act && pi >= 1) {
      const int v = pi - 1;
      double de[NE];
      if constexpr (AN) {
        pf_event_jac_col<Prob>(ph.phase_num, v, t0, x0, tf, xf, pp, c, de);
      } else {
#pragma unroll
        for (int i = 0; i < NE; ++i) de[i] = (ev[i] - base[i]) / h;
      }
      int pos;
      if (v < NX) pos = 2 * v;
      else if (v == NX) pos = 2 * NX;
      else if (v <= 2 * NX) pos = 2 * (v - NX - 1) + 1;
      else pos = v;
#pragma unroll
      for (int i = 0; i < NE; ++i)
        if (i < ph.ne) { vals[ph.v_evt0 + i * (2 * NX + 2 + NQ) + pos] = de[i]; chk_note(bad_j, de[i]); }
    }
  } else {
    const LinkDev lk = K.links[task.idx];
    const PhaseDev pl = K.phases[lk.left];
    const PhaseDev pr = K.phases[lk.right];
    const int pi = tid;
    const bool act = pi <= 2 * NX + 2 * NQ;
    double xl[NX], xr[NX], lo[NL], ql[NQs], qr[NQs];
#pragma unroll
    for (int j = 0; j < NQ; ++j) {
      ql[j] = x[pl.x_t0 + 2 + j];
      qr[j] = x[pr.x_t0 + 2 + j];
    }
#pragma unroll
    for (int j = 0; j < NX; ++j) {
      xl[j] = x[pl.x_state0 + j * (pl.N + 1) + pl.N];
      xr[j] = x[pr.x_state0 + j * (pr.N + 1)];
    }
    double h = 1.0;
    if (WJ && !AN && pi >= 1) {
      const int v = pi - 1;
#pragma unroll
      for (int j = 0; j < NX; ++j) {
        if (v == j) { h = K.tol * (1 + fabs(xl[j])); xl[j] += h; }
        if (v == NX + NQ + j) { h = K.tol * (1 + fabs(xr[j])); xr[j] += h; }
      }
#pragma unroll
      for (int j = 0; j < NQ; ++j) {
        if (v == NX + j) { h = K.tol * (1 + fabs(ql[j])); ql[j] += h; }
        if (v == 2 * NX + NQ + j) { h = K.tol * (1 + fabs(qr[j])); qr[j] += h; }
      }
    }
#pragma unroll
    for (int i = 0; i < NL; ++i) lo[i] = 0.0;
    if (act && (pi == 0 || !AN)) pf_link<Prob>(lk.left + 1, lk.right + 1, xl, xr, ql, qr, c, lk.nlink, lo);
    double base[NL];
    if constexpr (WAVE) {
#pragma unroll
      for (int i = 0; i < NL; ++i) base[i] = __shfl(lo[i], 0, 64);
    }
    if (pi == 0) {
#pragma unroll
      for (int i = 0; i < NL; ++i)
        if (i < lk.nlink) {
          if (!WAVE) lds[i] = lo[i];
          if (WG) { g[lk.g0 + i] = lo[i]; chk_note(bad_g, lo[i]); }
        }
    }
    if constexpr (!WAVE) {
      __syncthreads();
#pragma unroll
      for (int i = 0; i < NL; ++i) base[i] = lds[i];
    }
    if (WJ && act && pi >= 1) {
      const int v = pi - 1;
      double dl[NL];
      if constexpr (AN) {
        pf_link_jac_col<Prob>(lk.left + 1, lk.right + 1, v, xl, xr, ql, qr, c, lk.nlink, dl);
      } else {
#pragma unroll
        for (int i = 0; i < NL; ++i) dl[i] = (lo[i] - base[i]) / (1.0 * h);
      }
#pragma unroll
      for (int i = 0; i < NL; ++i)
        if (i < lk.nlink) { vals[lk.v0 + v * lk.nlink + i] = dl[i]; chk_note(bad_j, dl[i]); }
    }
  }
  chk_report(K.chk, bad_g, bad_j);
}


template <class Prob, bool WJ, bool AN, bool STG = false, class CP>
__device__ __forceinline__ void role_dynamics(int phase_num, int role, double tk, const double* xs, const double* us, CP c,
                                              double* f, double* cp,
                                              const typename stage_of<Prob>::type* base_stage = nullptr) {
  const int v = role - 1;
  if constexpr (STG) {
    Prob::dae_from(phase_num, tk, xs, us, c, *base_stage, (WJ && role >= 1) ? v : -1, f, cp);
  } else if (!AN || role == 0) {
    pf_dae<Prob>(phase_num, tk, xs, us, us + Prob::NU, c, f, cp);
  } else if constexpr (AN) {
    pf_dae_jac_col<Prob>(phase_num, v, tk, xs, us, us + Prob::NU, c, f, cp);
  }
}

template <int NX, int NU, int NQ>
__device__ __forceinline__ double perturb_uniform(int v, double pv, double tol, double* xs, double* us, double& tk) {
  const double h = tol * (1 + fabs(pv));
  const double pp = pv + h;
#pragma unroll
  for (int i = 0; i < NX; ++i) xs[i] = (v == i) ? pp : xs[i];
#pragma unroll
  for (int j = 0; j < NU; ++j) us[j] = (v == NX + j) ? pp : us[j];
  tk = (v == NX + NU) ? pp : tk;
#pragma unroll
  for (int j = 0; j < NQ; ++j) us[NU + j] = (v == NX + NU + 1 + j) ? pp : us[NU + j];
  return h;
}

template <class Prob, int T, bool WG, bool CHK>
__device__ __forceinline__ void publish_base(const double* f, const double* cp, double* Fb, int kk, double* g, int g0, int N,
                                             int k, bool& bad_g) {
  constexpr int NX = Prob::NX, NC = Prob::NC;
#pragma unroll
  for (int i = 0; i < NX; ++i) Fb[i * T + kk] = f[i];
#pragma unroll
  for (int j = 0; j < NC; ++j) {
    Fb[(NX + j) * T + kk] = cp[j];
    if (WG) {
      g[g0 + (NX + j) * N + k] = cp[j];
      if (CHK) chk_note(bad_g, cp[j]);
    }
  }
}

template <int T, bool CHK>
__device__ __forceinline__ void store_defect(int sv, double dx, double tspan, const double* Fb, int kk, double* g, int g0,
                                             int N, int k, bool& bad_g) {
  const double dfc = dx - Fb[sv * T + kk] * (tspan / 2.0);
  g[g0 + sv * N + k] = dfc;
  if (CHK) chk_note(bad_g, dfc);
}

__device__ __forceinline__ int xcd_place(int b, int count) {
  const int per = count >> 3, rem = count & 7, xcd = b & 7;
  return xcd * per + (xcd < rem ? xcd : rem) + (b >> 3);
}

#define RPM_REC(rec, f) __builtin_amdgcn_readfirstlane((rec)[offsetof(TileDev, f) / 4])

template <class Prob, int T, bool WG, bool WJ, bool AN, bool DXM = false>
__global__ void rpm_tile_kernel(const KParams K, const double* __restrict__ xall,
                                double* __restrict__ gall, double* __restrict__ vall) {
  constexpr int NX = Prob::NX, NU = Prob::NU, NC = Prob::NC, NQ = prob_nq<Prob>::value;
  constexpr int NO = NX + NC;
  constexpr int NV = NX + NU + 1 + NQ;
  constexpr int NB = NX + NU + 2 + NQ;
  constexpr int R = WJ ? NV + 1 : (NX > 0 ? NX : 1);
  constexpr int NCs = NC > 0 ? NC : 1;
  extern __shared__ double lds[];
  const int tid = threadIdx.x, nthr = blockDim.x;
  const double* __restrict__ x = xall + size_t(blockIdx.y) * K.n;
  double* __restrict__ g = gall + size_t(blockIdx.y) * K.sg;
  double* __restrict__ vals = vall + size_t(blockIdx.y) * K.sv;
  if (int(blockIdx.x) >= K.n_my_tiles) {
    endpoint_block<Prob, WG, WJ, AN>(K, K.tasks[int(blockIdx.x) - K.n_my_tiles], x, g, vals, lds, int(blockIdx.y));
    return;
  }
  const TileDev tl = K.tiles[xcd_place(int(blockIdx.x), K.n_my_tiles)];
  const TileDev& ph = tl;
  const auto c = (const __attribute__((address_space(4))) double*)(K.consts + size_t(blockIdx.y) * K.consts_stride);
  const TileLds L(NX, NU, NC, T, K.max_span, K.max_drow);
  double *Xs = lds + L.Xs, *Us = lds + L.Us, *Ds = lds + L.Ds, *Fb = lds + L.Fb, *DXs = lds + L.DXs;

  const int kk = tid % T, role = tid / T;
  bool bad_g = false, bad_j = false;
  const int kc = kk < tl.cnt ? kk : tl.cnt - 1;
  const int k = tl.k0 + kc;
  const int nidx = ph.node0 + k;
  const double tau = K.points[nidx];
  const NodeDev nd = K.nodes[nidx];
  const double ddiag = WJ ? K.diag[nidx] : 0.0;
  constexpr int CPRE = 8;
  double cpre[CPRE > 0 ? CPRE : 1];
  if (WJ && !K.skip_const) {
#pragma unroll
    for (int u = 0; u < CPRE; ++u) {
      const int q = tid + u * nthr;
      cpre[u] = q < tl.c_cnt ? K.doff_vals[tl.c_src0 + q] : 0.0;
    }
  }

  for (int q = tid; q < NX * tl.span_len; q += nthr) {
    const int i = q / tl.span_len, r = q - i * tl.span_len;
    Xs[i * K.max_span + r] = x[ph.x_state0 + i * (ph.N + 1) + tl.span0 + r];
  }
  for (int q = tid; q < NU * tl.cnt; q += nthr) {
    const int j = q / tl.cnt, r = q - j * tl.cnt;
    Us[j * T + r] = x[ph.x_control0 + j * ph.N + tl.k0 + r];
  }
  if (WG)
    for (int q = tid; q < tl.drow_len; q += nthr) Ds[q] = K.dvals[tl.drow0 + q];
  const double t0 = x[ph.x_t0], tf = x[ph.x_t0 + 1];
  __syncthreads();

  const bool act = kk < tl.cnt && role < R;
  const double tspan = tf - t0;
  double tk = (tau + 1) * (tspan / 2.0) + t0;
  double xs[NX > 0 ? NX : 1], us[NU + NQ > 0 ? NU + NQ : 1];
#pragma unroll
  for (int i = 0; i < NX; ++i) xs[i] = Xs[i * K.max_span + (k - tl.span0)];
#pragma unroll
  for (int j = 0; j < NU; ++j) us[j] = Us[j * T + kc];
#pragma unroll
  for (int j = 0; j < NQ; ++j) us[NU + j] = x[ph.x_t0 + 2 + j];

  const int sv = WJ ? role - 1 : role;
  double dx = 0.0;
  if (WG && !DXM && sv >= 0 && sv < NX) {
    const double* drow = Ds + (nd.drow_off - tl.drow0);
    const double* xcol = Xs + sv * K.max_span + (nd.dcol0 - tl.span0);
    for (int j = 0; j < nd.dlen; ++j) dx += drow[j] * xcol[j];
  }
  if constexpr (DXM && WG) {
    if (tid < 64) {
      typedef double d4 __attribute__((ext_vector_type(4)));
      const int lr = tid & 15, kq = tid >> 4;
      const int ksteps = (tl.span_len + 3) >> 2;
      for (int rb = 0; rb < T; rb += 16) {
        const int row = rb + lr;
        const bool row_ok = row < tl.cnt;
        const NodeDev ndr = K.nodes[ph.node0 + tl.k0 + (row_ok ? row : tl.cnt - 1)];
        const int rel0 = ndr.dcol0 - tl.span0;
        const double* drow = Ds + (ndr.drow_off - tl.drow0);
        for (int cb = 0; cb < NX; cb += 16) {
          const int st = cb + lr;
          d4 acc = {0.0, 0.0, 0.0, 0.0};
          for (int s = 0; s < ksteps; ++s) {
            const int kcol = 4 * s + kq;
            const int rel = kcol - rel0;
            const double a = (row_ok && rel >= 0 && rel < ndr.dlen) ? drow[rel] : 0.0;
            const double b = (st < NX && kcol < tl.span_len) ? Xs[st * K.max_span + kcol] : 0.0;
            acc = __builtin_amdgcn_mfma_f64_16x16x4f64(a, b, acc, 0, 0, 0);
          }
#pragma unroll
          for (int i = 0; i < 4; ++i) {
            const int orow = rb + kq + 4 * i;
            if (st < NX && orow < tl.cnt) DXs[st * T + orow] = acc[i];
          }
        }
      }
    }
  }

  double h = 1.0;
  const int v = role - 1;
  if (WJ && !AN && role >= 1) {
#pragma unroll
    for (int i = 0; i < NX; ++i)
      if (v == i) { h = K.tol * (1 + fabs(xs[i])); xs[i] += h; }
#pragma unroll
    for (int j = 0; j < NU; ++j)
      if (v == NX + j) { h = K.tol * (1 + fabs(us[j])); us[j] += h; }
    if (v == NX + NU) { h = K.tol * (1 + fabs(tk)); tk += h; }
#pragma unroll
    for (int j = 0; j < NQ; ++j)
      if (v == NX + NU + 1 + j) { h = K.tol * (1 + fabs(us[NU + j])); us[NU + j] += h; }
  }
  double f[NX > 0 ? NX : 1], cp[NCs];
  role_dynamics<Prob, WJ, AN>(ph.phase_num, role, tk, xs, us, c, f, cp);
  if (role == 0 && act) publish_base<Prob, T, WG, true>(f, cp, Fb, kk, g, ph.g0, ph.N, k, bad_g);
  __syncthreads();

  if (act) {
    const int N = ph.N;
    if (WG && sv >= 0 && sv < NX) store_defect<T, true>(sv, DXM ? DXs[sv * T + kk] : dx, tspan, Fb, kk, g, ph.g0, N, k, bad_g);
    if (WJ && role >= 1) {
      double J[NO];
#pragma unroll
      for (int o = 0; o < NO; ++o) {
        const double pert = o < NX ? f[o < NX ? o : 0] : cp[o >= NX ? o - NX : 0];
        J[o] = AN ? pert : (pert - Fb[o * T + kk]) / h;
      }
      double* vb = vals + ph.v_nl0 + k;
      if (v != NX + NU) {
        const int bv = v < NX + NU ? v : v + 1;
#pragma unroll
        for (int o = 0; o < NO; ++o) {
          double val;
          if (o < NX) {
            const double ret = J[o] * (tf - t0) / 2.0;
            val = (o == v) ? ddiag - ret : -ret;
          } else {
            val = J[o];
          }
          vb[size_t(o * NB + bv) * N] = val;
          chk_note(bad_j, val);
        }
      } else {
        const double a0 = -(tau * 0.5) + 0.5, af = (tau * 0.5) + 0.5;
#pragma unroll
        for (int o = 0; o < NO; ++o) {
          double v0, vf;
          if (o < NX) {
            const double fb = Fb[o * T + kk];
            const double dt = J[o] * (tf - t0) / 2.0;
            v0 = fb * (0.5) - a0 * dt;
            vf = -fb * (0.5) + af * dt;
          } else {
            v0 = a0 * J[o];
            vf = af * J[o];
          }
          vb[size_t(o * NB + NX + NU) * N] = v0;
          vb[size_t(o * NB + NX + NU + 1) * N] = vf;
          chk_note(bad_j, v0);
          chk_note(bad_j, vf);
        }
      }
    }
  }
  chk_report(K.chk, bad_g, bad_j);

  if (WJ && !K.skip_const) {
    const double* __restrict__ src = K.doff_vals + tl.c_src0;
    double* __restrict__ dst = vals + tl.c_dst0;
#pragma unroll
    for (int u = 0; u < CPRE; ++u) {
      const int q = tid + u * nthr;
      if (q < tl.c_cnt) {
#pragma unroll
        for (int i = 0; i < NX; ++i) dst[size_t(i) * tl.c_stride + q] = cpre[u];
      }
    }
    for (int q = tid + CPRE * nthr; q < tl.c_cnt; q += nthr) {
      const double dv = src[q];
#pragma unroll
      for (int i = 0; i < NX; ++i) dst[size_t(i) * tl.c_stride + q] = dv;
    }
  }
}

#ifdef RPM_DIAG
#define RPM_TRC(i)                                                                                            \
  if (K.trace && threadIdx.x == 0)                                                                            \
  K.trace[(size_t(blockIdx.y) * gridDim.x + blockIdx.x) * 8 + (i)] = wall_clock64()
#else
#define RPM_TRC(i)
#endif
template <class Prob, int T, int RG, bool WG, bool WJ, bool AN>
__global__ __launch_bounds__(T* RG) void rpm_tile_rl_kernel(const KParams K, const double* __restrict__ xall,
                                                            double* __restrict__ gall, double* __restrict__ vall) {
  constexpr int NX = Prob::NX, NU = Prob::NU, NC = Prob::NC, NQ = prob_nq<Prob>::value;
  constexpr int NO = NX + NC, NV = NX + NU + 1 + NQ, NB = NX + NU + 2 + NQ;
  constexpr int R = WJ ? NV + 1 : (NX > 0 ? NX : 1);
  constexpr int NCs = NC > 0 ? NC : 1;
  constexpr int NTHR = T * RG;
  extern __shared__ double lds[];
  const int tid = threadIdx.x;
  const double* __restrict__ x = xall + size_t(blockIdx.y) * K.n;
  double* __restrict__ g = gall + size_t(blockIdx.y) * K.sg;
  double* __restrict__ vals = vall + size_t(blockIdx.y) * K.sv;
  RPM_TRC(0);
  if (int(blockIdx.x) >= K.n_my_tiles) {
    endpoint_block<Prob, WG, WJ, AN>(K, K.tasks[int(blockIdx.x) - K.n_my_tiles], x, g, vals, lds, int(blockIdx.y));
    return;
  }
  const TileDev tl = K.tiles[xcd_place(int(blockIdx.x), K.n_my_tiles)];
  const TileDev& ph = tl;
  const auto c = (const __attribute__((address_space(4))) double*)(K.consts + size_t(blockIdx.y) * K.consts_stride);
  const TileLds L(NX, NU, NC, T, K.max_span, K.max_drow);
  double *Xs = lds + L.Xs, *Us = lds + L.Us, *Ds = lds + L.Ds, *Fb = lds + L.Fb;
  const int kk = tid % T, grp = __builtin_amdgcn_readfirstlane(tid / T);
  const int kc = kk < tl.cnt ? kk : tl.cnt - 1;
  const int k = tl.k0 + kc;
  const int nidx = ph.node0 + k;
  const double tau = K.points[nidx];
  const NodeDev nd = K.nodes[nidx];
  const double ddiag = WJ ? K.diag[nidx] : 0.0;
  for (int q = tid; q < NX * tl.span_len; q += NTHR) {
    const int i = q / tl.span_len, r = q - i * tl.span_len;
    Xs[i * K.max_span + r] = x[ph.x_state0 + i * (ph.N + 1) + tl.span0 + r];
  }
  for (int q = tid; q < NU * tl.cnt; q += NTHR) {
    const int j = q / tl.cnt, r = q - j * tl.cnt;
    Us[j * T + r] = x[ph.x_control0 + j * ph.N + tl.k0 + r];
  }
  if (WG)
    for (int q = tid; q < tl.drow_len; q += NTHR) Ds[q] = K.dvals[tl.drow0 + q];
  const double t0 = x[ph.x_t0], tf = x[ph.x_t0 + 1];
  RPM_TRC(1);
  __syncthreads();
  RPM_TRC(2);

  const bool node_ok = kk < tl.cnt;
  const double tspan = tf - t0;
  const double tk0 = (tau + 1) * (tspan / 2.0) + t0;
  const int N = ph.N;
  bool first = true, no_chk = false;
  for (int role = grp; role < R || first; role += RG) {
    const bool act = node_ok && role < R;
    double xs[NX > 0 ? NX : 1], us[NU + NQ > 0 ? NU + NQ : 1];
#pragma unroll
    for (int i = 0; i < NX; ++i) xs[i] = Xs[i * K.max_span + (k - tl.span0)];
#pragma unroll
    for (int j = 0; j < NU; ++j) us[j] = Us[j * T + kc];
#pragma unroll
    for (int j = 0; j < NQ; ++j) us[NU + j] = x[ph.x_t0 + 2 + j];
    double tk = tk0;
    const int sv = WJ ? role - 1 : role;
    double dx = 0.0;
    if (WG && sv >= 0 && sv < NX) {
      const double* drow = Ds + (nd.drow_off - tl.drow0);
      const double* xcol = Xs + sv * K.max_span + (nd.dcol0 - tl.span0);
      for (int j = 0; j < nd.dlen; ++j) dx += drow[j] * xcol[j];
    }
    double h = 1.0;
    const int v = role - 1;
    if (WJ && !AN && role >= 1) {
      double pv;
      if (v < NX) pv = Xs[v * K.max_span + (k - tl.span0)];
      else if (v < NX + NU) pv = Us[(v - NX) * T + kc];
      else if (v == NX + NU) pv = tk;
      else pv = x[ph.x_t0 + 1 + (v - NX - NU)];
      h = perturb_uniform<NX, NU, NQ>(v, pv, K.tol, xs, us, tk);
    }
    double f[NX > 0 ? NX : 1], cp[NCs];
    role_dynamics<Prob, WJ, AN>(ph.phase_num, role, tk, xs, us, c, f, cp);
    if (first) {
      if (role == 0 && act) publish_base<Prob, T, WG, false>(f, cp, Fb, kk, g, ph.g0, N, k, no_chk);
      __syncthreads();
      RPM_TRC(3);
      first = false;
    }
    if (act) {
      if (WG && sv >= 0 && sv < NX) store_defect<T, false>(sv, dx, tspan, Fb, kk, g, ph.g0, N, k, no_chk);
      if (WJ && role >= 1) {
        double J[NO];
#pragma unroll
        for (int o = 0; o < NO; ++o) {
          const double pert = o < NX ? f[o < NX ? o : 0] : cp[o >= NX ? o - NX : 0];
          J[o] = AN ? pert : (pert - Fb[o * T + kk]) / h;
        }
        double* vb = vals + ph.v_nl0 + k;
        if (v != NX + NU) {
          const int bv = v < NX + NU ? v : v + 1;
#pragma unroll
          for (int o = 0; o < NO; ++o) {
            double val;
            if (o < NX) {
              const double ret = J[o] * (tf - t0) / 2.0;
              val = (o == v) ? ddiag - ret : -ret;
            } else {
              val = J[o];
            }
            vb[size_t(o * NB + bv) * N] = val;
          }
        } else {
          const double a0 = -(tau * 0.5) + 0.5, af = (tau * 0.5) + 0.5;
#pragma unroll
          for (int o = 0; o < NO; ++o) {
            double v0, vf;
            if (o < NX) {
              const double fb = Fb[o * T + kk];
              const double dt = J[o] * (tf - t0) / 2.0;
              v0 = fb * (0.5) - a0 * dt;
              vf = -fb * (0.5) + af * dt;
            } else {
              v0 = a0 * J[o];
              vf = af * J[o];
            }
            vb[size_t(o * NB + NX + NU) * N] = v0;
            vb[size_t(o * NB + NX + NU + 1) * N] = vf;
          }
        }
      }
    }
  }
  RPM_TRC(4);
  if (WJ && !K.skip_const) {
    const double* __restrict__ src = K.doff_vals + tl.c_src0;
    double* __restrict__ dst = vals + tl.c_dst0;
    const int lead = int((reinterpret_cast<size_t>(dst) >> 3) & 15);
    for (int q = tid - lead; q < tl.c_cnt; q += NTHR) {
      if (q >= 0) {
        const double dv = src[q];
#pragma unroll
        for (int i = 0; i < NX; ++i) dst[size_t(i) * tl.c_stride + q] = dv;
      }
    }
  }
#ifdef RPM_DIAG
  RPM_TRC(5);
  if (K.trace) {
    __builtin_amdgcn_s_waitcnt(0);
    RPM_TRC(6);
    if (threadIdx.x == 0) {
      unsigned hw;
      asm volatile("s_getreg_b32 %0, hwreg(HW_REG_HW_ID)" : "=s"(hw));
      unsigned xcc;
      asm volatile("s_getreg_b32 %0, hwreg(HW_REG_XCC_ID)" : "=s"(xcc));
      K.trace[(size_t(blockIdx.y) * gridDim.x + blockIdx.x) * 8 + 7] = (static_cast<unsigned long long>(xcc) << 32) | hw;
    }
  }
#endif
}

constexpr int PL_CMAX = 1280, PL_REC = 32;
static_assert(sizeof(TileDev) / sizeof(int) < PL_REC, "tile record plus the instance index must fit the staged record");
static_assert(sizeof(TileDev) % 8 == 0, "the tile record is copied as doubles");

struct PlLds {
  int rec, next, tt, X, U, D, tau, diag, nodes, cv, stage;
  int Fb, ready, DXs, half;
  __host__ __device__ constexpr PlLds(int nx, int nu, int nc, int nq, int max_span, int max_drow, int max_cshare, bool with_jac,
                                      bool dxm)
      : rec(0), next(PL_REC / 2), tt(PL_REC), X(tt + 2 + ((nq + 1) & ~1)), U(X + nx * max_span), D(U + nu * 64),
        tau(D + max_drow), diag(tau + 64), nodes(diag + 64), cv(nodes + 2 * 64), stage(cv + (with_jac ? max_cshare : 0)),
        Fb(2 * stage), ready(Fb + (nx + nc) * 64), DXs(ready + 2), half(DXs + (dxm ? nx * 64 : 0)) {}
};
constexpr bool pl_lds_pinned(int nx, int nu, int nc, int nq, int span, int drow, int cshare, bool wj, bool dxm) {
  const PlLds L(nx, nu, nc, nq, span, drow, cshare, wj, dxm);
  const int nqe = (nq + 1) & ~1;
  return L.rec == 0 && L.next == L.rec + PL_REC / 2 && L.tt == L.next + PL_REC / 2 && L.X == L.tt + 2 + nqe &&
         L.U == L.X + nx * span && L.D == L.U + nu * 64 && L.tau == L.D + drow && L.diag == L.tau + 64 &&
         L.nodes == L.diag + 64 && L.cv == L.nodes + 2 * 64 && L.stage == L.cv + (wj ? cshare : 0) && L.Fb == 2 * L.stage &&
         L.ready == L.Fb + (nx + nc) * 64 && L.DXs == L.ready + 2 && L.half == L.DXs + (dxm ? nx * 64 : 0) &&
         L.stage == PL_REC + 2 + nqe + nx * span + nu * 64 + drow + 4 * 64 + (wj ? cshare : 0) &&
         L.half == 2 * L.stage + (nx + nc) * 64 + 2 + (dxm ? nx * 64 : 0);
}
static_assert(pl_lds_pinned(LaunchProblem::NX, LaunchProblem::NU, LaunchProblem::NC, 0, 73, 64 * 9, 1024, true, false) &&
                  pl_lds_pinned(LaunchProblem::NX, LaunchProblem::NU, LaunchProblem::NC, 1, 80, 64 * 17, 1280, true, true) &&
                  pl_lds_pinned(QuadrotorProblem::NX, QuadrotorProblem::NU, QuadrotorProblem::NC, 0, 65, 64 * 65, 640, false, true),
              "PlLds: an array overlaps its neighbour or a size changed");
typedef double d2u __attribute__((ext_vector_type(2), aligned(8)));
#define RPM_GPTR(p) ((const __attribute__((address_space(1))) void*)(p))
#define RPM_LPTR(p) ((__attribute__((address_space(3))) void*)(p))
template <int NPART>
__device__ __forceinline__ void pl_dma_run(const double* gsrc, double* ldst, int len, int lane, int part) {
  const int pairs = len >> 1;
#pragma unroll 1
  for (int ch = part; ch * 64 < pairs; ch += NPART)
    if (ch * 64 + lane < pairs)
      __builtin_amdgcn_global_load_lds(RPM_GPTR(gsrc + ch * 128 + 2 * lane), RPM_LPTR(ldst + ch * 128), 16, 0, 0);
  if ((len & 1) && part == 0 && lane < 2)
    __builtin_amdgcn_global_load_lds(RPM_GPTR(reinterpret_cast<const int*>(gsrc + len - 1) + lane),
                                     RPM_LPTR(ldst + len - 1), 4, 0, 0);
}


template <int NX, int NPART>
__device__ __forceinline__ void pl_const_stores(const double* cur, const double* cv_src, int inst_word, double* __restrict__ vall,
                                                long long sv, int lane, int part) {
  constexpr int CCH = (PL_CMAX / 128 + NPART - 1) / NPART;
  const int* rec = reinterpret_cast<const int*>(cur);
  const int c_dst0 = RPM_REC(rec, c_dst0);
  const int inst = __builtin_amdgcn_readfirstlane(rec[inst_word]);
  const int c_cnt = RPM_REC(rec, c_cnt);
  const int c_stride = RPM_REC(rec, c_stride);
  double* __restrict__ cdst = vall + size_t(inst) * sv + c_dst0;
  const int head = min(int((16 - ((reinterpret_cast<size_t>(cdst) >> 3) & 15)) & 15), c_cnt);
  d2u cv[CCH];
#pragma unroll
  for (int ch = 0; ch < CCH; ++ch) {
    const int q = max(min(head + (NPART * ch + part) * 128 + 2 * lane, c_cnt - 2), 0);
    cv[ch].x = cv_src[q];
    cv[ch].y = cv_src[q + 1];
  }
  const bool odd_tail = ((c_cnt - head) & 1) != 0;
  const int edge = lane < head ? lane : (lane == head && odd_tail ? c_cnt - 1 : -1);
  const double cedge = cv_src[max(edge, 0)];
#pragma unroll
  for (int ch = 0; ch < CCH; ++ch) {
    const int q = head + (NPART * ch + part) * 128 + 2 * lane;
    if (q + 1 < c_cnt) {
#pragma unroll
      for (int i = 0; i < NX; ++i) __builtin_nontemporal_store(cv[ch], reinterpret_cast<d2u*>(cdst + size_t(i) * c_stride + q));
    }
  }
  if (part == 0 && edge >= 0) {
#pragma unroll
    for (int i = 0; i < NX; ++i) cdst[size_t(i) * c_stride + edge] = cedge;
  }
}

constexpr int pl_role_groups(int R) { return (R + (R + 11) / 12 - 1) / ((R + 11) / 12); }

struct PlShape { int NH, RG, NDMA; };
constexpr PlShape pl_shape(int R) { return R <= 12 ? PlShape{2, 4, 2} : PlShape{1, pl_role_groups(R), 2}; }

template <class Prob, int NH, int RG, int NDMA, bool WG, bool WJ, bool AN, bool DXM = false, bool STG = false>
__global__ __launch_bounds__(NH * 64 * (RG + NDMA), 1) void rpm_tile_pl_kernel(
    const KParams K, int n_inst, const double* __restrict__ xall, double* __restrict__ gall,
    double* __restrict__ vall) {
  constexpr int T = 64;
  constexpr int HT = 64 * (RG + NDMA);
  constexpr int NX = Prob::NX, NU = Prob::NU, NC = Prob::NC, NQ = prob_nq<Prob>::value;
  constexpr int NXs = NX > 0 ? NX : 1, NUs = NU + NQ > 0 ? NU + NQ : 1;
  constexpr int NO = NX + NC, NV = NX + NU + 1 + NQ, NB = NX + NU + 2 + NQ;
  constexpr int R = WJ ? NV + 1 : (NX > 0 ? NX : 1);
  constexpr int NCs = NC > 0 ? NC : 1;
  constexpr int NTHR = T * RG;
  constexpr int NREC = int(sizeof(TileDev) / sizeof(int));
  extern __shared__ double lds_all[];
  const int half = NH > 1 ? __builtin_amdgcn_readfirstlane(int(threadIdx.x) / HT) : 0;
  const int tid = int(threadIdx.x) - half * HT;
  const int nb = int(gridDim.x), wg = xcd_place(int(blockIdx.x), nb);
  const int G = NH * nb, w = NH * wg + half;
  const int nt = K.n_my_tiles;
  const int W = nt * n_inst;
  const int n_iter = w < W ? (W - w + G - 1) / G : 0;
  const int n_iter_wg = (W - NH * wg + G - 1) / G;
  const PlLds L(NX, NU, NC, NQ, K.max_span, K.max_drow, K.max_cshare, WJ, DXM);
  const int S_TT = L.tt, S_X = L.X, S_U = L.U, S_D = L.D, S_TAU = L.tau, S_DG = L.diag, S_ND = L.nodes, S_CV = L.cv, S_SIZE = L.stage;
  double* lds = lds_all + half * L.half;
  double *Fb = lds + L.Fb, *DXs = lds + L.DXs;
  int* fb_ready = reinterpret_cast<int*>(lds + L.ready);
  int* dx_ready = fb_ready + 1;
#ifdef RPM_DIAG
#define RPM_PTRC(j, slot)                                                           \
  if (K.trace && (threadIdx.x & 63) == 0 && (j) < 2) K.trace[size_t(w) * 64 + (j)*32 + (slot)] = wall_clock64()
#define RPM_PEDGE(slot) \
  if (K.trace && (threadIdx.x & 63) == 0) K.trace[size_t(w) * 64 + (slot)] = wall_clock64()
#define RPM_PEDGE_MAX(slot) \
  if (K.trace && (threadIdx.x & 63) == 0) atomicMax(K.trace + size_t(w) * 64 + (slot), (unsigned long long)wall_clock64())
#else
#define RPM_PTRC(j, slot)
#define RPM_PEDGE(slot)
#define RPM_PEDGE_MAX(slot)
#endif
  if (tid == 0) { RPM_PTRC(0, 31); }

  struct TileRuns { int k0, cnt, span0, span_len, drow0, drow_len, N, x_state0, x_control0, x_t0, node0, c_src0, c_cnt; };
  auto runs_of = [&](auto p) {
    return TileRuns{RPM_REC(p, k0), RPM_REC(p, cnt), RPM_REC(p, span0), RPM_REC(p, span_len), RPM_REC(p, drow0),
                    RPM_REC(p, drow_len), RPM_REC(p, N), RPM_REC(p, x_state0), RPM_REC(p, x_control0), RPM_REC(p, x_t0),
                    RPM_REC(p, node0), RPM_REC(p, c_src0), RPM_REC(p, c_cnt)};
  };
  auto stage = [&](auto np_c, int part, int lane, int item, double* buf, const TileRuns tl) {
    constexpr int NP = decltype(np_c)::value;
    const int inst = item / nt, tidx = item - inst * nt;
    const double* __restrict__ x = xall + size_t(inst) * K.n;
    int rot = 0;
    auto run = [&](const double* gsrc, double* ldst, int len) {
      pl_dma_run<NP>(gsrc, ldst, len, lane, (part + NP - (rot++ % NP)) % NP);
    };
    if (part == 0 && lane == 0) reinterpret_cast<int*>(buf + L.rec)[NREC] = inst;
    run(reinterpret_cast<const double*>(K.tiles + tidx), buf + L.rec, NREC / 2);
    if (item + G < W) {
      const int item2 = item + G, inst2 = item2 / nt;
      run(reinterpret_cast<const double*>(K.tiles + (item2 - inst2 * nt)), buf + L.next, NREC / 2);
    }
    run(x + tl.x_t0, buf + S_TT, 2 + NQ);
#pragma unroll
    for (int i = 0; i < NX; ++i) run(x + tl.x_state0 + i * (tl.N + 1) + tl.span0, buf + S_X + i * K.max_span, tl.span_len);
#pragma unroll
    for (int j = 0; j < NU; ++j) run(x + tl.x_control0 + j * tl.N + tl.k0, buf + S_U + j * T, tl.cnt);
    run(K.points + tl.node0 + tl.k0, buf + S_TAU, tl.cnt);
    if (WJ) run(K.diag + tl.node0 + tl.k0, buf + S_DG, tl.cnt);
    run(reinterpret_cast<const double*>(K.nodes + tl.node0 + tl.k0), buf + S_ND, 2 * tl.cnt);
    if (WG) run(K.dvals + tl.drow0, buf + S_D, tl.drow_len);
    if (WJ && !K.skip_const) run(K.doff_vals + tl.c_src0, buf + S_CV, tl.c_cnt);
  };
  const auto first_runs = [&]() { return runs_of((const __attribute__((address_space(4))) int*)(K.tiles + (w - (w / nt) * nt))); };
  if (tid >= NTHR) {
    const int lane = (tid - NTHR) & 63;
    const int dw = __builtin_amdgcn_readfirstlane((tid - NTHR) >> 6);
    __builtin_amdgcn_s_setprio(3);
    if (dw == 0 && lane == 0) { *fb_ready = 0; *dx_ready = 0; }
    {
      const auto r0 = first_runs();
      RPM_PTRC(0, 19);
      if (n_iter > 0) stage(std::integral_constant<int, NDMA>{}, dw, lane, w, lds, r0);
      RPM_PTRC(0, 20);
    }
#ifdef RPM_DIAG
    unsigned long long wait_sum = 0, wait_max = 0;
#endif
    for (int j = 0; j < n_iter_wg; ++j) {
      const double* cur = lds + (j & 1) * S_SIZE;
      double* nxt = lds + ((j + 1) & 1) * S_SIZE;
#ifdef RPM_DIAG
      const unsigned long long tw0 = wall_clock64();
#endif
      __builtin_amdgcn_s_waitcnt(0);
#ifdef RPM_DIAG
      const unsigned long long tw = wall_clock64() - tw0;
      wait_sum += tw;
      wait_max = tw > wait_max ? tw : wait_max;
#endif
      __syncthreads();
      RPM_PTRC(j, 16);
      if constexpr (DXM && WG) {
        if (j < n_iter) {
          typedef double d4 __attribute__((ext_vector_type(4)));
          const int* rec = reinterpret_cast<const int*>(cur + L.rec);
          const int cnt = RPM_REC(rec, cnt);
          const int span0 = RPM_REC(rec, span0);
          const int drow0 = RPM_REC(rec, drow0);
          const NodeDev* ND = reinterpret_cast<const NodeDev*>(cur + S_ND);
          const double* Ds = cur + S_D;
          const double* Xs = cur + S_X;
          const int lr = lane & 15, kq = lane >> 4;
          for (int rb = 16 * dw; rb < cnt; rb += 16 * NDMA) {
            const int row = rb + lr;
            const bool row_ok = row < cnt;
            const NodeDev ndr = ND[row_ok ? row : cnt - 1];
            const int rel0 = ndr.dcol0 - span0;
            const double* drow = Ds + (ndr.drow_off - drow0);
            const NodeDev nfirst = ND[rb], nlast = ND[min(rb + 15, cnt - 1)];
            const int kmin = __builtin_amdgcn_readfirstlane(nfirst.dcol0 - span0);
            const int kmax = __builtin_amdgcn_readfirstlane(nlast.dcol0 + nlast.dlen - span0);
            for (int cb = 0; cb < NX; cb += 16) {
              const int st = cb + lr;
              d4 acc = {0.0, 0.0, 0.0, 0.0};
              for (int k0 = kmin; k0 < kmax; k0 += 4) {
                const int kcol = k0 + kq;
                const int rel = kcol - rel0;
                const double a = (row_ok && rel >= 0 && rel < ndr.dlen) ? drow[rel] : 0.0;
                const double b = (st < NX && kcol < kmax) ? Xs[st * K.max_span + kcol] : 0.0;
                acc = __builtin_amdgcn_mfma_f64_16x16x4f64(a, b, acc, 0, 0, 0);
              }
#pragma unroll
              for (int i = 0; i < 4; ++i) {
                const int orow = rb + kq + 4 * i;
                if (st < NX && orow < cnt) DXs[st * T + orow] = acc[i];
              }
            }
          }
          if (lane == 0) __hip_atomic_fetch_add(dx_ready, 1, __ATOMIC_RELEASE, __HIP_MEMORY_SCOPE_WORKGROUP);
        }
      }
      if (WJ && !K.skip_const && j < n_iter) pl_const_stores<NX, NDMA>(cur + L.rec, cur + S_CV, NREC, vall, K.sv, lane, dw);
      RPM_PTRC(j, 17);
      if (j + 1 < n_iter) {
        stage(std::integral_constant<int, NDMA>{}, dw, lane, w + (j + 1) * G, nxt, runs_of(reinterpret_cast<const int*>(cur + L.next)));
      }
      RPM_PTRC(j, 18);
    }
#ifdef RPM_DIAG
    if (K.trace && lane == 0 && n_iter > 0) {
      K.trace[size_t(w) * 64 + 28 + dw] = wait_sum;
      K.trace[size_t(w) * 64 + 32 + 28 + dw] = wait_max;
    }
#endif
    const int n_end = K.n_tasks * n_inst;
    for (int it = NDMA * w + dw; it < n_end; it += NDMA * G) {
      const int inst = it / K.n_tasks;
      endpoint_block<Prob, WG, WJ, AN, true>(K, K.tasks[it - inst * K.n_tasks], xall + size_t(inst) * K.n,
                                             gall + size_t(inst) * K.sg, vall + size_t(inst) * K.sv, nullptr, inst);
    }
    return;
  }

  const int kk = tid % T, grp = __builtin_amdgcn_readfirstlane(tid / T);
  for (int jt = 0; jt < n_iter_wg; ++jt) {
    const double* cur = lds + (jt & 1) * S_SIZE;
    asm volatile("s_waitcnt lgkmcnt(0)\n\ts_barrier" ::: "memory");
    if (jt >= n_iter) continue;
    if (grp < 4) { RPM_PTRC(jt, grp * 4 + 0); }
    if (grp == 0 && jt == n_iter - 1) { RPM_PEDGE(22); }
    const int* rec = reinterpret_cast<const int*>(cur + L.rec);
    const int k0 = RPM_REC(rec, k0);
    const int cnt = RPM_REC(rec, cnt);
    const int span0 = RPM_REC(rec, span0);
    const int drow0 = RPM_REC(rec, drow0);
    const int N = RPM_REC(rec, N);
    const int phase_num = RPM_REC(rec, phase_num);
    const int g0 = RPM_REC(rec, g0);
    const int v_nl0 = RPM_REC(rec, v_nl0);
    const int inst = __builtin_amdgcn_readfirstlane(rec[NREC]);
    double* __restrict__ g = gall + size_t(inst) * K.sg;
    double* __restrict__ vals = vall + size_t(inst) * K.sv;
    const auto c4 = (const __attribute__((address_space(4))) double*)(K.consts + size_t(inst) * K.consts_stride);
    const double* Xs = cur + S_X;
    const double* Us = cur + S_U;
    const double* Ds = cur + S_D;
    const int kc = kk < cnt ? kk : cnt - 1;
    const int k = k0 + kc;
    const bool node_ok = kk < cnt;
    bool first = true, no_chk = false;
    typename stage_of<Prob>::type base_stage;
    if constexpr (STG) {
      static_assert(NQ == 0 && !AN, "staged evaluation: finite differences, no static parameters");
      double xs0[NXs], us0[NUs];
#pragma unroll
      for (int i = 0; i < NX; ++i) xs0[i] = Xs[i * K.max_span + (k - span0)];
#pragma unroll
      for (int j = 0; j < NU; ++j) us0[j] = Us[j * T + kc];
      const double tau0 = cur[S_TAU + kc], t00 = cur[S_TT], tf0 = cur[S_TT + 1];
      Prob::stage(phase_num, (tau0 + 1) * ((tf0 - t00) / 2.0) + t00, xs0, us0, c4, base_stage);
    }
    for (int role = grp; role < R || first; role += RG) {
      const bool act = node_ok && role < R;
#ifdef RPM_DIAG
      const bool trc = role == 5;
      if (trc) { RPM_PTRC(jt, 24); }
#endif
      double xs[NXs], us[NUs];
#pragma unroll
      for (int i = 0; i < NX; ++i) xs[i] = Xs[i * K.max_span + (k - span0)];
#pragma unroll
      for (int j = 0; j < NU; ++j) us[j] = Us[j * T + kc];
#pragma unroll
      for (int j = 0; j < NQ; ++j) us[NU + j] = cur[S_TT + 2 + j];
      double tk;
      {
        const double tau = cur[S_TAU + kc], t0 = cur[S_TT], tf = cur[S_TT + 1];
        tk = (tau + 1) * ((tf - t0) / 2.0) + t0;
      }
      const int sv = WJ ? role - 1 : role;
      double dx = 0.0;
      if (WG && !DXM && sv >= 0 && sv < NX) {
        const NodeDev nd = reinterpret_cast<const NodeDev*>(cur + S_ND)[kc];
        const double* drow = Ds + (nd.drow_off - drow0);
        const double* xcol = Xs + sv * K.max_span + (nd.dcol0 - span0);
        int j = 0;
        for (; j + 4 <= nd.dlen; j += 4) {
          const double d0 = drow[j], d1 = drow[j + 1], d2 = drow[j + 2], d3 = drow[j + 3];
          const double x0 = xcol[j], x1 = xcol[j + 1], x2 = xcol[j + 2], x3 = xcol[j + 3];
          dx += d0 * x0;
          dx += d1 * x1;
          dx += d2 * x2;
          dx += d3 * x3;
        }
        for (; j < nd.dlen; ++j) dx += drow[j] * xcol[j];
      }
#ifdef RPM_DIAG
      if (trc) { if (dx == 1e300) xs[0] = 0; RPM_PTRC(jt, 25); }
#endif
      double h = 1.0;
      const int v = role - 1;
      if (WJ && !AN && role >= 1) {
        double pv;
        if (v < NX) pv = Xs[v * K.max_span + (k - span0)];
        else if (v < NX + NU) pv = Us[(v - NX) * T + kc];
        else if (v == NX + NU) pv = tk;
        else pv = cur[S_TT + 1 + (v - NX - NU)];
        h = perturb_uniform<NX, NU, NQ>(v, pv, K.tol, xs, us, tk);
      }
      double f[NXs], cp[NCs];
      role_dynamics<Prob, WJ, AN, STG>(phase_num, role, tk, xs, us, c4, f, cp, &base_stage);
#ifdef RPM_DIAG
      if (trc) { if (f[0] == 1e300) cp[0] = 0; RPM_PTRC(jt, 26); }
#endif
      if (first) {
        if (role == 0 && act) publish_base<Prob, T, WG, false>(f, cp, Fb, kk, g, g0, N, k, no_chk);
        if (grp < 4) { RPM_PTRC(jt, grp * 4 + 1); }
        if (grp == 0) {
          __hip_atomic_store(fb_ready, jt + 1, __ATOMIC_RELEASE, __HIP_MEMORY_SCOPE_WORKGROUP);
        } else {
          while (__hip_atomic_load(fb_ready, __ATOMIC_ACQUIRE, __HIP_MEMORY_SCOPE_WORKGROUP) < jt + 1)
            __builtin_amdgcn_s_sleep(1);
        }
        if (grp < 4) { RPM_PTRC(jt, grp * 4 + 2); }
        first = false;
      }
      if (act) {
        const double tau = cur[S_TAU + kc], t0 = cur[S_TT], tf = cur[S_TT + 1];
        const double ddiag = cur[S_DG + kc];
        if (WG && sv >= 0 && sv < NX) {
          if constexpr (DXM) {
            while (__hip_atomic_load(dx_ready, __ATOMIC_ACQUIRE, __HIP_MEMORY_SCOPE_WORKGROUP) < NDMA * (jt + 1)) __builtin_amdgcn_s_sleep(1);
            dx = DXs[sv * T + kk];
          }
          store_defect<T, false>(sv, dx, tf - t0, Fb, kk, g, g0, N, k, no_chk);
        }
        if (WJ && role >= 1) {
          double J[NO];
#pragma unroll
          for (int o = 0; o < NO; ++o) {
            const double pert = o < NX ? f[o < NX ? o : 0] : cp[o >= NX ? o - NX : 0];
            J[o] = AN ? pert : (pert - Fb[o * T + kk]) / h;
          }
          double* __restrict__ vb = vals + v_nl0;
          if (v != NX + NU) {
            const int bv = v < NX + NU ? v : v + 1;
#pragma unroll
            for (int o = 0; o < NO; ++o) {
              double val;
              if (o < NX) {
                const double ret = J[o] * (tf - t0) / 2.0;
                val = (o == v) ? ddiag - ret : -ret;
              } else {
                val = J[o];
              }
              (vb + size_t(o * NB + bv) * N)[k] = val;
            }
          } else {
            const double a0 = -(tau * 0.5) + 0.5, af = (tau * 0.5) + 0.5;
#pragma unroll
            for (int o = 0; o < NO; ++o) {
              double v0, vf;
              if (o < NX) {
                const double fb = Fb[o * T + kk];
                const double dt = J[o] * (tf - t0) / 2.0;
                v0 = fb * (0.5) - a0 * dt;
                vf = -fb * (0.5) + af * dt;
              } else {
                v0 = a0 * J[o];
                vf = af * J[o];
              }
              (vb + size_t(o * NB + NX + NU) * N)[k] = v0;
              (vb + size_t(o * NB + NX + NU + 1) * N)[k] = vf;
            }
          }
        }
      }
#ifdef RPM_DIAG
      if (trc) { RPM_PTRC(jt, 27); }
#endif
    }
    if (grp < 4) { RPM_PTRC(jt, grp * 4 + 3); }
    if (jt == n_iter - 1) { RPM_PEDGE_MAX(23); }
  }
}

static size_t pl_lds_bytes(int nx, int nu, int nc, int nq, const KParams& kp, bool dxm) {
  const PlLds L(nx, nu, nc, nq, kp.max_span, kp.max_drow, kp.max_cshare, true, dxm);
  return size_t(pl_shape(nx + nu + 2 + nq).NH) * L.half * sizeof(double);
}

void tile_pipeline_setup(Engine& e, Device* d, const ProblemDims& pd, int device_id) {
    int ncu = 0;
    if (hipDeviceGetAttribute(&ncu, hipDeviceAttributeMultiprocessorCount, device_id) != hipSuccess || ncu <= 0) ncu = 256;
    const int max_c = d->kp.max_cshare;
    int per_cu = 0;
    with_problem(e.problem_id, [&](auto prob) {
      using P = decltype(prob);
      constexpr PlShape S = pl_shape(P::NX + P::NU + 2 + prob_nq<P>::value);
      d->pl_lds = pl_lds_bytes(pd.nx, pd.nu, pd.nc, pd.nq, d->kp, false);
      if (d->pl_lds > 160 * 1024) return;
      auto kern = rpm_tile_pl_kernel<P, S.NH, S.RG, S.NDMA, true, true, false>;
      if (d->pl_lds > 64 * 1024)
        (void)hipFuncSetAttribute(reinterpret_cast<const void*>(kern), hipFuncAttributeMaxDynamicSharedMemorySize,
                                  int(d->pl_lds));
      if (hipOccupancyMaxActiveBlocksPerMultiprocessor(&per_cu, kern, S.NH * 64 * (S.RG + S.NDMA), d->pl_lds) != hipSuccess)
        per_cu = 0;
      (void)hipGetLastError();
      per_cu *= S.NH;
    });
    d->pl_slots = per_cu * ncu;
    d->pl_ok = e.role_looped && e.tile_nodes == 64 && max_c <= PL_CMAX && max_c >= 2 && 2 * pd.nx + 3 + 2 * pd.nq <= 64 &&
               per_cu >= 1;
}

template <class Kern>
static hipError_t allow_lds(Kern kern, size_t bytes) {
  if (bytes <= 64 * 1024) return hipSuccess;
  return hipFuncSetAttribute(reinterpret_cast<const void*>(kern), hipFuncAttributeMaxDynamicSharedMemorySize, int(bytes));
}

template <class Kern>
static hipError_t launch_tiles(const Engine& e, Kern kern, int threads, const KParams& kp, const double* dx, double* dg,
                               double* dv, hipStream_t st) {
  const Device& d = *e.dev;
  hipError_t s = allow_lds(kern, d.lds_bytes);
  if (s != hipSuccess) return s;
  dim3 grid(unsigned(d.kp.n_my_tiles + d.kp.n_tasks), unsigned(e.n_instances));
  if (grid.x == 0) return hipSuccess;
  hipLaunchKernelGGL(kern, grid, dim3(threads), d.lds_bytes, st, kp, dx, dg, dv);
  return hipGetLastError();
}

static bool pl_dxm_ok(const Engine& e) {
  ProblemDims pd;
  problem_dims(e.problem_id, &pd);
  return e.first_derive != RPM_DERIVE_ANALYTIC && pl_lds_bytes(pd.nx, pd.nu, pd.nc, pd.nq, e.dev->kp, true) <= 160 * 1024;
}

template <class Prob, bool WG, bool WJ, bool AN, bool DXM, bool STG = false>
static hipError_t launch_tile_pl(const Engine& e, const KParams& kp, const double* dx, double* dg, double* dv, hipStream_t st) {
  if constexpr (!STG && !AN && has_stage<Prob>::value) {
    if (e.opt_stage_roles == 1 || (e.opt_stage_roles < 0 && (kp.skip_const || stage_always<Prob>::value)))
      return launch_tile_pl<Prob, WG, WJ, AN, DXM, true>(e, kp, dx, dg, dv, st);
  }
  const Device& d = *e.dev;
  constexpr PlShape S = pl_shape(Prob::NX + Prob::NU + 2 + prob_nq<Prob>::value);
  auto kern = rpm_tile_pl_kernel<Prob, S.NH, S.RG, S.NDMA, WG, WJ, AN, DXM, STG>;
  const size_t lds = pl_lds_bytes(Prob::NX, Prob::NU, Prob::NC, prob_nq<Prob>::value, d.kp, DXM);
  hipError_t s = allow_lds(kern, lds);
  if (s != hipSuccess) return s;
  const long long W = (long long)d.kp.n_my_tiles * e.n_instances;
  const long long halves = W < d.pl_slots ? W : d.pl_slots;
  hipLaunchKernelGGL(kern, dim3(unsigned((halves + S.NH - 1) / S.NH)), dim3(S.NH * 64 * (S.RG + S.NDMA)), lds, st, kp,
                     e.n_instances, dx, dg, dv);
  return hipGetLastError();
}

static bool use_pipeline(const Engine& e) {
  const Device& d = *e.dev;
  if (!d.pl_ok || e.opt_pipeline == 0 || d.kp.n_my_tiles <= 0) return false;
  if (e.opt_pipeline == 1) return true;
  const long long W = (long long)d.kp.n_my_tiles * e.n_instances;
  return W >= 2LL * d.pl_slots || (W <= d.pl_slots && 4 * W >= 3LL * d.pl_slots);
}

static int cons_layout(const Engine& e) {
  if (!(e.role_looped && e.tile_nodes == 64)) return 0;
  if (e.opt_dx_mode == 0) return use_pipeline(e) ? 2 : 1;
  return (use_pipeline(e) && pl_dxm_ok(e)) ? 2 : 0;
}
bool dev_cons_is_one_role(const Engine& e) { return !e.dev || cons_layout(e) == 0; }

int dev_pipeline_active(const Engine& e) { return e.dev && cons_layout(e) == 2 ? 1 : 0; }

template <bool WG_, bool WJ_, bool AN_, bool DXM_>
struct TileFlags { static constexpr bool WG = WG_, WJ = WJ_, AN = AN_, DXM = DXM_; };

template <class Prob, class Launch>
static hipError_t with_tile_flags(const Engine& e, bool wg, bool wj, Launch&& launch) {
  if constexpr (Prob::HAS_ANALYTIC) {
    if (wj && e.first_derive == RPM_DERIVE_ANALYTIC)
      return wg ? launch(TileFlags<true, true, true, false>{}) : launch(TileFlags<false, true, true, false>{});
  }
  if (wg && e.opt_dx_mode == 1)
    return wj ? launch(TileFlags<true, true, false, true>{}) : launch(TileFlags<true, false, false, true>{});
  if (wg && wj) return launch(TileFlags<true, true, false, false>{});
  if (wj) return launch(TileFlags<false, true, false, false>{});
  return launch(TileFlags<true, false, false, false>{});
}

template <class Prob, int T>
static hipError_t launch_tile_T(const Engine& e, const KParams& kp, bool wg, bool wj, const double* dx, double* dg,
                                double* dv, hipStream_t st) {
  const int layout = T == 64 ? cons_layout(e) : 0;
  return with_tile_flags<Prob>(e, wg, wj, [&](auto flags) -> hipError_t {
    using F = decltype(flags);
    if constexpr (T == 64) {
      if (layout == 2) return launch_tile_pl<Prob, F::WG, F::WJ, F::AN, F::DXM>(e, kp, dx, dg, dv, st);
      if constexpr (!F::DXM) {
        if (layout == 1) return launch_tiles(e, rpm_tile_rl_kernel<Prob, 64, 4, F::WG, F::WJ, F::AN>, 64 * 4, kp, dx, dg, dv, st);
      }
    }
    constexpr int R = F::WJ ? Prob::NX + Prob::NU + 2 + prob_nq<Prob>::value : (Prob::NX > 0 ? Prob::NX : 1);
    constexpr int threads = (T * R + 63) / 64 * 64;
    return launch_tiles(e, rpm_tile_kernel<Prob, T, F::WG, F::WJ, F::AN, F::DXM>, threads, kp, dx, dg, dv, st);
  });
}

int dev_eval_cons(Engine& e, const double* d_x, double* d_g, double* d_values, int flags, void* stream) {
  if (!e.dev) {
    int rc = device_init(e, 0);
    if (rc) return rc;
  }
  hipStream_t st = static_cast<hipStream_t>(stream);
  const bool wg = flags & 1, wj = flags & 2;
  KParams kp = e.dev->kp;
  kp.sg = (flags & 4) ? e.stride_g() : e.m;
  kp.sv = (flags & 4) ? e.stride_values() : e.nnz_jac;
  kp.chk = ((flags & 8) && dev_cons_is_one_role(e)) ? e.dev->d_flags2 : nullptr;
  kp.skip_const = 0;
  if (wj && (flags & 16) && d_values) {
    auto& seen = e.dev->const_filled;
    if (std::find(seen.begin(), seen.end(), d_values) != seen.end()) {
      kp.skip_const = 1;
    } else {
      if (seen.size() >= 4096) seen.clear();
      seen.push_back(d_values);
    }
  }
  hipError_t s = hipErrorInvalidValue;
  with_problem(e.problem_id, [&](auto prob) {
    using P = decltype(prob);
    switch (e.tile_nodes) {
      case 64: s = launch_tile_T<P, 64>(e, kp, wg, wj, d_x, d_g, d_values, st); break;
      case 32: s = launch_tile_T<P, 32>(e, kp, wg, wj, d_x, d_g, d_values, st); break;
      default: s = launch_tile_T<P, 16>(e, kp, wg, wj, d_x, d_g, d_values, st); break;
    }
  });
  if (s != hipSuccess) {
    e.err = std::string("rpm_tile_kernel launch: ") + hipGetErrorString(s);
    return RPM_E_DEVICE;
  }
  return RPM_OK;
}

}
```

Measured before the change: 631,400.

## Keep mesh tables resident in LDS when each pipeline slot always sees one tile

Splits the pipelined kernel's LDS staging into a mesh part (tile record, D values, tau, diag, nodes, constants) and a per-instance part (x slice, controls, times). When the grid size makes each slot revisit the same tile across instances, the mesh part is staged once and only instance data is re-fetched each iteration. The first iteration's constant-share loads are also waited on late through partial vmcnt. This cuts repeated global-to-LDS traffic but adds layout complexity, a runtime branch on residency, and padded x loads that may read one element past the end.

```diff
diff --git a/lpopc_amd/csrc/rpm_abi.cpp b/lpopc_amd/csrc/rpm_abi.cpp
--- a/lpopc_amd/csrc/rpm_abi.cpp
+++ b/lpopc_amd/csrc/rpm_abi.cpp
@@ -617,6 +617,7 @@
   else if (k == "dx_mode") *value = e.opt_dx_mode;
   else if (k == "tile_nodes") *value = e.tile_nodes;
   else if (k == "n_tiles") *value = int(e.tiles.size());
+  else if (k == "max_span") *value = e.max_span;
   else if (k == "role_loop") *value = e.role_looped ? 1 : 0;
   else if (k == "pipeline") *value = e.opt_pipeline;
   else if (k == "mesh_err_tile") *value = e.opt_mesh_err_tile;
@@ -646,6 +647,7 @@
   else if (k == "stride_g") *value = int(e.stride_g());
   else if (k == "stride_values") *value = int(e.stride_values());
   else if (k == "pipeline_active") *value = rpm::dev_pipeline_active(e);
+  else if (k == "pipeline_resident") *value = rpm::dev_pipeline_resident(e);
   else return fail(e, RPM_E_INVALID, "unknown option");
   return RPM_OK;
 }
diff --git a/lpopc_amd/csrc/rpm_device.hip b/lpopc_amd/csrc/rpm_device.hip
--- a/lpopc_amd/csrc/rpm_device.hip
+++ b/lpopc_amd/csrc/rpm_device.hip
@@ -287,6 +287,7 @@
   k.tasks = d->d_tasks;
   k.n_tasks = (!sharded || e.shard_rank == 0) ? int(e.tasks.size()) : 0;
   k.skip_const = 0;
+  k.pl_resident = 0;
   k.trace = nullptr;
   k.chk = nullptr;
 #ifdef RPM_DIAG
diff --git a/lpopc_amd/csrc/rpm_device_internal.hpp b/lpopc_amd/csrc/rpm_device_internal.hpp
--- a/lpopc_amd/csrc/rpm_device_internal.hpp
+++ b/lpopc_amd/csrc/rpm_device_internal.hpp
@@ -41,6 +41,7 @@
   int max_span, max_drow;
   int max_cshare;
   int skip_const;
+  int pl_resident;
   unsigned long long* trace;
   int* chk;
 };
diff --git a/lpopc_amd/csrc/rpm_engine.hpp b/lpopc_amd/csrc/rpm_engine.hpp
--- a/lpopc_amd/csrc/rpm_engine.hpp
+++ b/lpopc_amd/csrc/rpm_engine.hpp
@@ -228,6 +228,7 @@
 int host_cons_end(Engine& e, double* g, double* values, const ConsCall& c, const char* who);
 int host_delta_sent_runs(Engine& e, int* sent);
 int dev_pipeline_active(const Engine& e);
+int dev_pipeline_resident(const Engine& e);
 int dev_upload_x(Engine& e, const double* x);
 int dev_upload(Engine& e, double* dev, const double* host, size_t count, int slot);
 int dev_download(Engine& e, double* host, const double* dev, size_t count, int slot);
diff --git a/lpopc_amd/csrc/rpm_tile_kernels.hip b/lpopc_amd/csrc/rpm_tile_kernels.hip
--- a/lpopc_amd/csrc/rpm_tile_kernels.hip
+++ b/lpopc_amd/csrc/rpm_tile_kernels.hip
@@ -580,55 +580,84 @@
 }
 
 constexpr int PL_CMAX = 1280, PL_REC = 32;
-static_assert(sizeof(TileDev) / sizeof(int) < PL_REC, "tile record plus the instance index must fit the staged record");
+static_assert(sizeof(TileDev) / sizeof(int) < PL_REC, "the tile record must fit its slot");
 static_assert(sizeof(TileDev) % 8 == 0, "the tile record is copied as doubles");
 
 struct PlLds {
-  int rec, next, tt, X, U, D, tau, diag, nodes, cv, stage;
-  int Fb, ready, DXs, half;
+  int rec, next, D, tau, diag, nodes, cv, mesh;
+  int xs, inst, tt, X, U, tile;
+  int n_mesh, tile0, Fb, ready, DXs, half;
   __host__ __device__ constexpr PlLds(int nx, int nu, int nc, int nq, int max_span, int max_drow, int max_cshare, bool with_jac,
-                                      bool dxm)
-      : rec(0), next(PL_REC / 2), tt(PL_REC), X(tt + 2 + ((nq + 1) & ~1)), U(X + nx * max_span), D(U + nu * 64),
-        tau(D + max_drow), diag(tau + 64), nodes(diag + 64), cv(nodes + 2 * 64), stage(cv + (with_jac ? max_cshare : 0)),
-        Fb(2 * stage), ready(Fb + (nx + nc) * 64), DXs(ready + 2), half(DXs + (dxm ? nx * 64 : 0)) {}
+                                      bool dxm, bool resident)
+      : rec(0), next(PL_REC / 2), D(next + (resident ? 0 : PL_REC / 2)), tau(D + max_drow), diag(tau + 64), nodes(diag + 64),
+        cv(nodes + 2 * 64), mesh(cv + (with_jac ? max_cshare : 0)),
+        xs((max_span + 1) & ~1), inst(0), tt(2), X(tt + 2 + ((nq + 1) & ~1)), U(X + nx * xs), tile(U + nu * 64),
+        n_mesh(resident ? 1 : 2), tile0(n_mesh * mesh), Fb(tile0 + 2 * tile), ready(Fb + (nx + nc) * 64), DXs(ready + 2),
+        half(DXs + (dxm ? nx * 64 : 0)) {}
 };
-constexpr bool pl_lds_pinned(int nx, int nu, int nc, int nq, int span, int drow, int cshare, bool wj, bool dxm) {
-  const PlLds L(nx, nu, nc, nq, span, drow, cshare, wj, dxm);
-  const int nqe = (nq + 1) & ~1;
-  return L.rec == 0 && L.next == L.rec + PL_REC / 2 && L.tt == L.next + PL_REC / 2 && L.X == L.tt + 2 + nqe &&
-         L.U == L.X + nx * span && L.D == L.U + nu * 64 && L.tau == L.D + drow && L.diag == L.tau + 64 &&
-         L.nodes == L.diag + 64 && L.cv == L.nodes + 2 * 64 && L.stage == L.cv + (wj ? cshare : 0) && L.Fb == 2 * L.stage &&
+constexpr bool pl_lds_pinned(int nx, int nu, int nc, int nq, int span, int drow, int cshare, bool wj, bool dxm, bool res) {
+  const PlLds L(nx, nu, nc, nq, span, drow, cshare, wj, dxm, res);
+  const int nqe = (nq + 1) & ~1, xs = span + (span & 1), nm = res ? 1 : 2;
+  return L.rec == 0 && L.next == L.rec + PL_REC / 2 && L.D == L.next + (res ? 0 : PL_REC / 2) && L.tau == L.D + drow &&
+         L.diag == L.tau + 64 && L.nodes == L.diag + 64 && L.cv == L.nodes + 2 * 64 && L.mesh == L.cv + (wj ? cshare : 0) &&
+         L.xs == xs && L.inst == 0 && L.tt == L.inst + 2 && L.X == L.tt + 2 + nqe && L.U == L.X + nx * xs &&
+         L.tile == L.U + nu * 64 && L.n_mesh == nm && L.tile0 == nm * L.mesh && L.Fb == L.tile0 + 2 * L.tile &&
          L.ready == L.Fb + (nx + nc) * 64 && L.DXs == L.ready + 2 && L.half == L.DXs + (dxm ? nx * 64 : 0) &&
-         L.stage == PL_REC + 2 + nqe + nx * span + nu * 64 + drow + 4 * 64 + (wj ? cshare : 0) &&
-         L.half == 2 * L.stage + (nx + nc) * 64 + 2 + (dxm ? nx * 64 : 0);
-}
-static_assert(pl_lds_pinned(LaunchProblem::NX, LaunchProblem::NU, LaunchProblem::NC, 0, 73, 64 * 9, 1024, true, false) &&
-                  pl_lds_pinned(LaunchProblem::NX, LaunchProblem::NU, LaunchProblem::NC, 1, 80, 64 * 17, 1280, true, true) &&
-                  pl_lds_pinned(QuadrotorProblem::NX, QuadrotorProblem::NU, QuadrotorProblem::NC, 0, 65, 64 * 65, 640, false, true),
+         L.mesh == (res ? 1 : 2) * (PL_REC / 2) + drow + 4 * 64 + (wj ? cshare : 0) &&
+         L.tile == 4 + nqe + nx * xs + nu * 64 &&
+         L.half == nm * L.mesh + 2 * L.tile + (nx + nc) * 64 + 2 + (dxm ? nx * 64 : 0);
+}
+constexpr bool pl_lds_pinned2(int nx, int nu, int nc, int nq, int span, int drow, int cshare, bool wj, bool dxm) {
+  return pl_lds_pinned(nx, nu, nc, nq, span, drow, cshare, wj, dxm, false) && pl_lds_pinned(nx, nu, nc, nq, span, drow, cshare, wj, dxm, true);
+}
+static_assert(pl_lds_pinned2(LaunchProblem::NX, LaunchProblem::NU, LaunchProblem::NC, 0, 73, 64 * 9, 1024, true, false) &&
+                  pl_lds_pinned2(LaunchProblem::NX, LaunchProblem::NU, LaunchProblem::NC, 1, 80, 64 * 17, 1280, true, true) &&
+                  pl_lds_pinned2(QuadrotorProblem::NX, QuadrotorProblem::NU, QuadrotorProblem::NC, 0, 65, 64 * 65, 640, false, true),
               "PlLds: an array overlaps its neighbour or a size changed");
+static_assert(PlLds(LaunchProblem::NX, LaunchProblem::NU, LaunchProblem::NC, 0, 73, 64 * 9, 1024, true, false, true).tile ==
+                  4 + LaunchProblem::NX * 74 + LaunchProblem::NU * 64,
+              "PlLds: the tile buffer holds only what depends on the instance");
 typedef double d2u __attribute__((ext_vector_type(2), aligned(8)));
 #define RPM_GPTR(p) ((const __attribute__((address_space(1))) void*)(p))
 #define RPM_LPTR(p) ((__attribute__((address_space(3))) void*)(p))
 template <int NPART>
-__device__ __forceinline__ void pl_dma_run(const double* gsrc, double* ldst, int len, int lane, int part) {
-  const int pairs = len >> 1;
+__device__ __forceinline__ int pl_dma_run(const double* gsrc, double* ldst, int len, int lane, int part, bool pad_ok = false) {
+  const int pairs = (len + (pad_ok ? 1 : 0)) >> 1;
+  int issued = 0;
 #pragma unroll 1
-  for (int ch = part; ch * 64 < pairs; ch += NPART)
+  for (int ch = part; ch * 64 < pairs; ch += NPART) {
     if (ch * 64 + lane < pairs)
       __builtin_amdgcn_global_load_lds(RPM_GPTR(gsrc + ch * 128 + 2 * lane), RPM_LPTR(ldst + ch * 128), 16, 0, 0);
-  if ((len & 1) && part == 0 && lane < 2)
-    __builtin_amdgcn_global_load_lds(RPM_GPTR(reinterpret_cast<const int*>(gsrc + len - 1) + lane),
-                                     RPM_LPTR(ldst + len - 1), 4, 0, 0);
+    ++issued;
+  }
+  if ((len & 1) && !pad_ok && part == 0) {
+    if (lane < 2)
+      __builtin_amdgcn_global_load_lds(RPM_GPTR(reinterpret_cast<const int*>(gsrc + len - 1) + lane),
+                                       RPM_LPTR(ldst + len - 1), 4, 0, 0);
+    ++issued;
+  }
+  return issued;
+}
+
+__device__ __forceinline__ void pl_wait_vmcnt(int n) {
+  switch (n) {
+    case 1: asm volatile("s_waitcnt vmcnt(1)" ::: "memory"); break;
+    case 2: asm volatile("s_waitcnt vmcnt(2)" ::: "memory"); break;
+    case 3: asm volatile("s_waitcnt vmcnt(3)" ::: "memory"); break;
+    case 4: asm volatile("s_waitcnt vmcnt(4)" ::: "memory"); break;
+    case 5: asm volatile("s_waitcnt vmcnt(5)" ::: "memory"); break;
+    case 6: asm volatile("s_waitcnt vmcnt(6)" ::: "memory"); break;
+    default: asm volatile("s_waitcnt vmcnt(0)" ::: "memory"); break;
+  }
 }
 
 
 template <int NX, int NPART>
-__device__ __forceinline__ void pl_const_stores(const double* cur, const double* cv_src, int inst_word, double* __restrict__ vall,
+__device__ __forceinline__ void pl_const_stores(const double* cur, const double* cv_src, int inst, double* __restrict__ vall,
                                                 long long sv, int lane, int part) {
   constexpr int CCH = (PL_CMAX / 128 + NPART - 1) / NPART;
   const int* rec = reinterpret_cast<const int*>(cur);
   const int c_dst0 = RPM_REC(rec, c_dst0);
-  const int inst = __builtin_amdgcn_readfirstlane(rec[inst_word]);
   const int c_cnt = RPM_REC(rec, c_cnt);
   const int c_stride = RPM_REC(rec, c_stride);
   double* __restrict__ cdst = vall + size_t(inst) * sv + c_dst0;
@@ -684,12 +713,15 @@
   const int W = nt * n_inst;
   const int n_iter = w < W ? (W - w + G - 1) / G : 0;
   const int n_iter_wg = (W - NH * wg + G - 1) / G;
-  const PlLds L(NX, NU, NC, NQ, K.max_span, K.max_drow, K.max_cshare, WJ, DXM);
-  const int S_TT = L.tt, S_X = L.X, S_U = L.U, S_D = L.D, S_TAU = L.tau, S_DG = L.diag, S_ND = L.nodes, S_CV = L.cv, S_SIZE = L.stage;
+  const bool resident = K.pl_resident != 0;
+  const PlLds L(NX, NU, NC, NQ, K.max_span, K.max_drow, K.max_cshare, WJ, DXM, resident);
+  const int S_TT = L.tt, S_X = L.X, S_U = L.U, XS = L.xs, S_TILE0 = L.tile0, S_TILE = L.tile;
+  const int S_D = L.D, S_TAU = L.tau, S_DG = L.diag, S_ND = L.nodes, S_CV = L.cv, S_MESH = resident ? 0 : L.mesh;
   double* lds = lds_all + half * L.half;
   double *Fb = lds + L.Fb, *DXs = lds + L.DXs;
   int* fb_ready = reinterpret_cast<int*>(lds + L.ready);
   int* dx_ready = fb_ready + 1;
+  int* cv_ready = fb_ready + 2;
 #ifdef RPM_DIAG
 #define RPM_PTRC(j, slot)                                                           \
   if (K.trace && (threadIdx.x & 63) == 0 && (j) < 2) K.trace[size_t(w) * 64 + (j)*32 + (slot)] = wall_clock64()
@@ -710,69 +742,83 @@
                     RPM_REC(p, drow_len), RPM_REC(p, N), RPM_REC(p, x_state0), RPM_REC(p, x_control0), RPM_REC(p, x_t0),
                     RPM_REC(p, node0), RPM_REC(p, c_src0), RPM_REC(p, c_cnt)};
   };
-  auto stage = [&](auto np_c, int part, int lane, int item, double* buf, const TileRuns tl) {
+  auto stage = [&](auto np_c, int part, int lane, int item, double* mbuf, double* tbuf, const TileRuns tl, bool mesh) -> int {
     constexpr int NP = decltype(np_c)::value;
     const int inst = item / nt, tidx = item - inst * nt;
     const double* __restrict__ x = xall + size_t(inst) * K.n;
     int rot = 0;
     auto run = [&](const double* gsrc, double* ldst, int len) {
-      pl_dma_run<NP>(gsrc, ldst, len, lane, (part + NP - (rot++ % NP)) % NP);
+      return pl_dma_run<NP>(gsrc, ldst, len, lane, (part + NP - (rot++ % NP)) % NP);
     };
-    if (part == 0 && lane == 0) reinterpret_cast<int*>(buf + L.rec)[NREC] = inst;
-    run(reinterpret_cast<const double*>(K.tiles + tidx), buf + L.rec, NREC / 2);
-    if (item + G < W) {
-      const int item2 = item + G, inst2 = item2 / nt;
-      run(reinterpret_cast<const double*>(K.tiles + (item2 - inst2 * nt)), buf + L.next, NREC / 2);
-    }
-    run(x + tl.x_t0, buf + S_TT, 2 + NQ);
-#pragma unroll
-    for (int i = 0; i < NX; ++i) run(x + tl.x_state0 + i * (tl.N + 1) + tl.span0, buf + S_X + i * K.max_span, tl.span_len);
-#pragma unroll
-    for (int j = 0; j < NU; ++j) run(x + tl.x_control0 + j * tl.N + tl.k0, buf + S_U + j * T, tl.cnt);
-    run(K.points + tl.node0 + tl.k0, buf + S_TAU, tl.cnt);
-    if (WJ) run(K.diag + tl.node0 + tl.k0, buf + S_DG, tl.cnt);
-    run(reinterpret_cast<const double*>(K.nodes + tl.node0 + tl.k0), buf + S_ND, 2 * tl.cnt);
-    if (WG) run(K.dvals + tl.drow0, buf + S_D, tl.drow_len);
-    if (WJ && !K.skip_const) run(K.doff_vals + tl.c_src0, buf + S_CV, tl.c_cnt);
+    auto run_x = [&](int at, double* ldst, int len) {
+      pl_dma_run<NP>(x + at, ldst, len, lane, (part + NP - (rot++ % NP)) % NP, at + len < K.n);
+    };
+    if (part == 0 && lane == 0) *reinterpret_cast<int*>(tbuf + L.inst) = inst;
+    if (mesh) {
+      run(reinterpret_cast<const double*>(K.tiles + tidx), mbuf + L.rec, NREC / 2);
+      if (!resident && item + G < W) {
+        const int item2 = item + G, inst2 = item2 / nt;
+        run(reinterpret_cast<const double*>(K.tiles + (item2 - inst2 * nt)), mbuf + L.next, NREC / 2);
+      }
+    }
+    run_x(tl.x_t0, tbuf + S_TT, 2 + NQ);
+#pragma unroll
+    for (int i = 0; i < NX; ++i) run_x(tl.x_state0 + i * (tl.N + 1) + tl.span0, tbuf + S_X + i * XS, tl.span_len);
+#pragma unroll
+    for (int j = 0; j < NU; ++j) run_x(tl.x_control0 + j * tl.N + tl.k0, tbuf + S_U + j * T, tl.cnt);
+    if (!mesh) return 0;
+    run(K.points + tl.node0 + tl.k0, mbuf + S_TAU, tl.cnt);
+    if (WJ) run(K.diag + tl.node0 + tl.k0, mbuf + S_DG, tl.cnt);
+    run(reinterpret_cast<const double*>(K.nodes + tl.node0 + tl.k0), mbuf + S_ND, 2 * tl.cnt);
+    if (WG) run(K.dvals + tl.drow0, mbuf + S_D, tl.drow_len);
+    if (WJ && !K.skip_const) return run(K.doff_vals + tl.c_src0, mbuf + S_CV, tl.c_cnt);
+    return 0;
   };
   const auto first_runs = [&]() { return runs_of((const __attribute__((address_space(4))) int*)(K.tiles + (w - (w / nt) * nt))); };
   if (tid >= NTHR) {
     const int lane = (tid - NTHR) & 63;
     const int dw = __builtin_amdgcn_readfirstlane((tid - NTHR) >> 6);
     __builtin_amdgcn_s_setprio(3);
-    if (dw == 0 && lane == 0) { *fb_ready = 0; *dx_ready = 0; }
+    if (dw == 0 && lane == 0) { *fb_ready = 0; *dx_ready = 0; *cv_ready = 0; }
+    int share_loads = 0;
     {
       const auto r0 = first_runs();
       RPM_PTRC(0, 19);
-      if (n_iter > 0) stage(std::integral_constant<int, NDMA>{}, dw, lane, w, lds, r0);
+      if (n_iter > 0) share_loads = stage(std::integral_constant<int, NDMA>{}, dw, lane, w, lds, lds + S_TILE0, r0, true);
       RPM_PTRC(0, 20);
     }
+    const bool share_late = resident && WJ && !K.skip_const && n_iter > 0;
 #ifdef RPM_DIAG
     unsigned long long wait_sum = 0, wait_max = 0;
 #endif
     for (int j = 0; j < n_iter_wg; ++j) {
-      const double* cur = lds + (j & 1) * S_SIZE;
-      double* nxt = lds + ((j + 1) & 1) * S_SIZE;
+      const double* cur = lds + S_TILE0 + (j & 1) * S_TILE;
+      const double* msh = lds + (j & 1) * S_MESH;
+      double* nxt = lds + S_TILE0 + ((j + 1) & 1) * S_TILE;
+      double* nxt_msh = lds + ((j + 1) & 1) * S_MESH;
+      const bool late = share_late && j == 0;
 #ifdef RPM_DIAG
       const unsigned long long tw0 = wall_clock64();
 #endif
-      __builtin_amdgcn_s_waitcnt(0);
+      if (late) pl_wait_vmcnt(share_loads);
+      else __builtin_amdgcn_s_waitcnt(0);
 #ifdef RPM_DIAG
       const unsigned long long tw = wall_clock64() - tw0;
       wait_sum += tw;
       wait_max = tw > wait_max ? tw : wait_max;
 #endif
-      __syncthreads();
+      if (late) asm volatile("s_waitcnt lgkmcnt(0)\n\ts_barrier" ::: "memory");
+      else __syncthreads();
       RPM_PTRC(j, 16);
       if constexpr (DXM && WG) {
         if (j < n_iter) {
           typedef double d4 __attribute__((ext_vector_type(4)));
-          const int* rec = reinterpret_cast<const int*>(cur + L.rec);
+          const int* rec = reinterpret_cast<const int*>(msh + L.rec);
           const int cnt = RPM_REC(rec, cnt);
           const int span0 = RPM_REC(rec, span0);
           const int drow0 = RPM_REC(rec, drow0);
-          const NodeDev* ND = reinterpret_cast<const NodeDev*>(cur + S_ND);
-          const double* Ds = cur + S_D;
+          const NodeDev* ND = reinterpret_cast<const NodeDev*>(msh + S_ND);
+          const double* Ds = msh + S_D;
           const double* Xs = cur + S_X;
           const int lr = lane & 15, kq = lane >> 4;
           for (int rb = 16 * dw; rb < cnt; rb += 16 * NDMA) {
@@ -791,7 +837,7 @@
                 const int kcol = k0 + kq;
                 const int rel = kcol - rel0;
                 const double a = (row_ok && rel >= 0 && rel < ndr.dlen) ? drow[rel] : 0.0;
-                const double b = (st < NX && kcol < kmax) ? Xs[st * K.max_span + kcol] : 0.0;
+                const double b = (st < NX && kcol < kmax) ? Xs[st * XS + kcol] : 0.0;
                 acc = __builtin_amdgcn_mfma_f64_16x16x4f64(a, b, acc, 0, 0, 0);
               }
 #pragma unroll
@@ -804,10 +850,18 @@
           if (lane == 0) __hip_atomic_fetch_add(dx_ready, 1, __ATOMIC_RELEASE, __HIP_MEMORY_SCOPE_WORKGROUP);
         }
       }
-      if (WJ && !K.skip_const && j < n_iter) pl_const_stores<NX, NDMA>(cur + L.rec, cur + S_CV, NREC, vall, K.sv, lane, dw);
+      if (late) {
+        asm volatile("s_waitcnt vmcnt(0)" ::: "memory");
+        if (lane == 0) __hip_atomic_fetch_add(cv_ready, 1, __ATOMIC_RELEASE, __HIP_MEMORY_SCOPE_WORKGROUP);
+        while (__hip_atomic_load(cv_ready, __ATOMIC_ACQUIRE, __HIP_MEMORY_SCOPE_WORKGROUP) < NDMA) __builtin_amdgcn_s_sleep(1);
+      }
+      if (WJ && !K.skip_const && j < n_iter)
+        pl_const_stores<NX, NDMA>(msh + L.rec, msh + S_CV, __builtin_amdgcn_readfirstlane(*reinterpret_cast<const int*>(cur + L.inst)),
+                                  vall, K.sv, lane, dw);
       RPM_PTRC(j, 17);
       if (j + 1 < n_iter) {
-        stage(std::integral_constant<int, NDMA>{}, dw, lane, w + (j + 1) * G, nxt, runs_of(reinterpret_cast<const int*>(cur + L.next)));
+        stage(std::integral_constant<int, NDMA>{}, dw, lane, w + (j + 1) * G, nxt_msh, nxt,
+              runs_of(reinterpret_cast<const int*>(msh + (resident ? L.rec : L.next))), !resident);
       }
       RPM_PTRC(j, 18);
     }
@@ -828,12 +882,13 @@
 
   const int kk = tid % T, grp = __builtin_amdgcn_readfirstlane(tid / T);
   for (int jt = 0; jt < n_iter_wg; ++jt) {
-    const double* cur = lds + (jt & 1) * S_SIZE;
+    const double* cur = lds + S_TILE0 + (jt & 1) * S_TILE;
+    const double* msh = lds + (jt & 1) * S_MESH;
     asm volatile("s_waitcnt lgkmcnt(0)\n\ts_barrier" ::: "memory");
     if (jt >= n_iter) continue;
     if (grp < 4) { RPM_PTRC(jt, grp * 4 + 0); }
     if (grp == 0 && jt == n_iter - 1) { RPM_PEDGE(22); }
-    const int* rec = reinterpret_cast<const int*>(cur + L.rec);
+    const int* rec = reinterpret_cast<const int*>(msh + L.rec);
     const int k0 = RPM_REC(rec, k0);
     const int cnt = RPM_REC(rec, cnt);
     const int span0 = RPM_REC(rec, span0);
@@ -842,13 +897,13 @@
     const int phase_num = RPM_REC(rec, phase_num);
     const int g0 = RPM_REC(rec, g0);
     const int v_nl0 = RPM_REC(rec, v_nl0);
-    const int inst = __builtin_amdgcn_readfirstlane(rec[NREC]);
+    const int inst = __builtin_amdgcn_readfirstlane(*reinterpret_cast<const int*>(cur + L.inst));
     double* __restrict__ g = gall + size_t(inst) * K.sg;
     double* __restrict__ vals = vall + size_t(inst) * K.sv;
     const auto c4 = (const __attribute__((address_space(4))) double*)(K.consts + size_t(inst) * K.consts_stride);
     const double* Xs = cur + S_X;
     const double* Us = cur + S_U;
-    const double* Ds = cur + S_D;
+    const double* Ds = msh + S_D;
     const int kc = kk < cnt ? kk : cnt - 1;
     const int k = k0 + kc;
     const bool node_ok = kk < cnt;
@@ -858,10 +913,10 @@
       static_assert(NQ == 0 && !AN, "staged evaluation: finite differences, no static parameters");
       double xs0[NXs], us0[NUs];
 #pragma unroll
-      for (int i = 0; i < NX; ++i) xs0[i] = Xs[i * K.max_span + (k - span0)];
+      for (int i = 0; i < NX; ++i) xs0[i] = Xs[i * XS + (k - span0)];
 #pragma unroll
       for (int j = 0; j < NU; ++j) us0[j] = Us[j * T + kc];
-      const double tau0 = cur[S_TAU + kc], t00 = cur[S_TT], tf0 = cur[S_TT + 1];
+      const double tau0 = msh[S_TAU + kc], t00 = cur[S_TT], tf0 = cur[S_TT + 1];
       Prob::stage(phase_num, (tau0 + 1) * ((tf0 - t00) / 2.0) + t00, xs0, us0, c4, base_stage);
     }
     for (int role = grp; role < R || first; role += RG) {
@@ -872,22 +927,22 @@
 #endif
       double xs[NXs], us[NUs];
 #pragma unroll
-      for (int i = 0; i < NX; ++i) xs[i] = Xs[i * K.max_span + (k - span0)];
+      for (int i = 0; i < NX; ++i) xs[i] = Xs[i * XS + (k - span0)];
 #pragma unroll
       for (int j = 0; j < NU; ++j) us[j] = Us[j * T + kc];
 #pragma unroll
       for (int j = 0; j < NQ; ++j) us[NU + j] = cur[S_TT + 2 + j];
       double tk;
       {
-        const double tau = cur[S_TAU + kc], t0 = cur[S_TT], tf = cur[S_TT + 1];
+        const double tau = msh[S_TAU + kc], t0 = cur[S_TT], tf = cur[S_TT + 1];
         tk = (tau + 1) * ((tf - t0) / 2.0) + t0;
       }
       const int sv = WJ ? role - 1 : role;
       double dx = 0.0;
       if (WG && !DXM && sv >= 0 && sv < NX) {
-        const NodeDev nd = reinterpret_cast<const NodeDev*>(cur + S_ND)[kc];
+        const NodeDev nd = reinterpret_cast<const NodeDev*>(msh + S_ND)[kc];
         const double* drow = Ds + (nd.drow_off - drow0);
-        const double* xcol = Xs + sv * K.max_span + (nd.dcol0 - span0);
+        const double* xcol = Xs + sv * XS + (nd.dcol0 - span0);
         int j = 0;
         for (; j + 4 <= nd.dlen; j += 4) {
           const double d0 = drow[j], d1 = drow[j + 1], d2 = drow[j + 2], d3 = drow[j + 3];
@@ -906,7 +961,7 @@
       const int v = role - 1;
       if (WJ && !AN && role >= 1) {
         double pv;
-        if (v < NX) pv = Xs[v * K.max_span + (k - span0)];
+        if (v < NX) pv = Xs[v * XS + (k - span0)];
         else if (v < NX + NU) pv = Us[(v - NX) * T + kc];
         else if (v == NX + NU) pv = tk;
         else pv = cur[S_TT + 1 + (v - NX - NU)];
@@ -930,8 +985,8 @@
         first = false;
       }
       if (act) {
-        const double tau = cur[S_TAU + kc], t0 = cur[S_TT], tf = cur[S_TT + 1];
-        const double ddiag = cur[S_DG + kc];
+        const double tau = msh[S_TAU + kc], t0 = cur[S_TT], tf = cur[S_TT + 1];
+        const double ddiag = msh[S_DG + kc];
         if (WG && sv >= 0 && sv < NX) {
           if constexpr (DXM) {
             while (__hip_atomic_load(dx_ready, __ATOMIC_ACQUIRE, __HIP_MEMORY_SCOPE_WORKGROUP) < NDMA * (jt + 1)) __builtin_amdgcn_s_sleep(1);
@@ -989,8 +1044,8 @@
   }
 }
 
-static size_t pl_lds_bytes(int nx, int nu, int nc, int nq, const KParams& kp, bool dxm) {
-  const PlLds L(nx, nu, nc, nq, kp.max_span, kp.max_drow, kp.max_cshare, true, dxm);
+static size_t pl_lds_bytes(int nx, int nu, int nc, int nq, const KParams& kp, bool dxm, bool resident) {
+  const PlLds L(nx, nu, nc, nq, kp.max_span, kp.max_drow, kp.max_cshare, true, dxm, resident);
   return size_t(pl_shape(nx + nu + 2 + nq).NH) * L.half * sizeof(double);
 }
 
@@ -1002,7 +1057,7 @@
     with_problem(e.problem_id, [&](auto prob) {
       using P = decltype(prob);
       constexpr PlShape S = pl_shape(P::NX + P::NU + 2 + prob_nq<P>::value);
-      d->pl_lds = pl_lds_bytes(pd.nx, pd.nu, pd.nc, pd.nq, d->kp, false);
+      d->pl_lds = pl_lds_bytes(pd.nx, pd.nu, pd.nc, pd.nq, d->kp, false, false);
       if (d->pl_lds > 160 * 1024) return;
       auto kern = rpm_tile_pl_kernel<P, S.NH, S.RG, S.NDMA, true, true, false>;
       if (d->pl_lds > 64 * 1024)
@@ -1039,7 +1094,16 @@
 static bool pl_dxm_ok(const Engine& e) {
   ProblemDims pd;
   problem_dims(e.problem_id, &pd);
-  return e.first_derive != RPM_DERIVE_ANALYTIC && pl_lds_bytes(pd.nx, pd.nu, pd.nc, pd.nq, e.dev->kp, true) <= 160 * 1024;
+  return e.first_derive != RPM_DERIVE_ANALYTIC && pl_lds_bytes(pd.nx, pd.nu, pd.nc, pd.nq, e.dev->kp, true, false) <= 160 * 1024;
+}
+
+struct PlGrid { int wgs; bool resident; };
+static PlGrid pl_grid(const Engine& e, int NH) {
+  const Device& d = *e.dev;
+  const long long W = (long long)d.kp.n_my_tiles * e.n_instances;
+  const long long halves = W < d.pl_slots ? W : d.pl_slots;
+  const int wgs = int((halves + NH - 1) / NH);
+  return PlGrid{wgs, wgs > 0 && (NH * wgs) % d.kp.n_my_tiles == 0};
 }
 
 template <class Prob, bool WG, bool WJ, bool AN, bool DXM, bool STG = false>
@@ -1051,13 +1115,13 @@
   const Device& d = *e.dev;
   constexpr PlShape S = pl_shape(Prob::NX + Prob::NU + 2 + prob_nq<Prob>::value);
   auto kern = rpm_tile_pl_kernel<Prob, S.NH, S.RG, S.NDMA, WG, WJ, AN, DXM, STG>;
-  const size_t lds = pl_lds_bytes(Prob::NX, Prob::NU, Prob::NC, prob_nq<Prob>::value, d.kp, DXM);
+  const PlGrid grid = pl_grid(e, S.NH);
+  KParams kpl = kp;
+  kpl.pl_resident = grid.resident ? 1 : 0;
+  const size_t lds = pl_lds_bytes(Prob::NX, Prob::NU, Prob::NC, prob_nq<Prob>::value, d.kp, DXM, grid.resident);
   hipError_t s = allow_lds(kern, lds);
   if (s != hipSuccess) return s;
-  const long long W = (long long)d.kp.n_my_tiles * e.n_instances;
-  const long long halves = W < d.pl_slots ? W : d.pl_slots;
-  hipLaunchKernelGGL(kern, dim3(unsigned((halves + S.NH - 1) / S.NH)), dim3(S.NH * 64 * (S.RG + S.NDMA)), lds, st, kp,
-                     e.n_instances, dx, dg, dv);
+  hipLaunchKernelGGL(kern, dim3(unsigned(grid.wgs)), dim3(S.NH * 64 * (S.RG + S.NDMA)), lds, st, kpl, e.n_instances, dx, dg, dv);
   return hipGetLastError();
 }
 
@@ -1077,6 +1141,13 @@
 bool dev_cons_is_one_role(const Engine& e) { return !e.dev || cons_layout(e) == 0; }
 
 int dev_pipeline_active(const Engine& e) { return e.dev && cons_layout(e) == 2 ? 1 : 0; }
+
+int dev_pipeline_resident(const Engine& e) {
+  if (!dev_pipeline_active(e)) return 0;
+  ProblemDims pd;
+  problem_dims(e.problem_id, &pd);
+  return pl_grid(e, pl_shape(pd.nx + pd.nu + 2 + pd.nq).NH).resident ? 1 : 0;
+}
 
 template <bool WG_, bool WJ_, bool AN_, bool DXM_>
 struct TileFlags { static constexpr bool WG = WG_, WJ = WJ_, AN = AN_, DXM = DXM_; };
```

Result: slower. 613,500 (-2.8%).
